# Farama-Foundation/Miniworld

Hardware: AMD Instinct MI355X
Metric: env-steps/s (batched, 80x60 RGB) (higher is better)
Workload: dtype f32

## Files before the change

include/mwengine.h:

```cpp
#ifndef MWENGINE_H
#define MWENGINE_H
#include <stdint.h>
#ifdef __cplusplus
extern "C" {
#endif

#define MW_ABI_VERSION 4

enum {
    MW_OK = 0,
    MW_E_INVALID = -1,
    MW_E_HIP = -2,
    MW_E_NOMEM = -3,
    MW_E_CAPACITY = -4,
    MW_E_DEVICE = -5,
    MW_E_OVERFLOW = -6
};

enum { MW_ENT_NONE = 0, MW_ENT_BOX = 1, MW_ENT_MESH = 2, MW_ENT_FRAME = 3 };

enum {
    MW_TASK_NONE = 0,
    MW_TASK_GOTO = 1,
    MW_TASK_PICKUP = 2,
// ... 236 lines not shown
    double cell;
    double margin;
    double reach;
    int32_t gx, gz;
    int32_t flags;
    int32_t target_slot;
} mw_nav_params;
int mw_nav_build(mw_engine *e, const mw_nav_params *params, const uint8_t *d_mask, const double *d_target, uint16_t *d_field, void *stream);
int mw_nav_query(mw_engine *e, const mw_nav_params *params, const double *d_target, const uint16_t *d_field, const double *d_pos,
                 int32_t *d_cost, int32_t *d_next, double *d_waypoint, void *stream);
int mw_debug_set_nav_passes(mw_engine *e, int32_t *d_passes);

#define MW_RAY_ENTITIES 1
#define MW_RAY_ENT 0x10000
#define MW_RAY_MAX 4096
typedef struct mw_ray_params {
    double max_t;
    double radius;
    int32_t rays;
    int32_t flags;
} mw_ray_params;
int mw_ray_cast(mw_engine *e, const mw_ray_params *params, const uint8_t *d_mask,
                const double *d_origin  ,
                const double *d_dir     ,
                const double *d_offsets ,
                double *d_t , int32_t *d_hit , double *d_dir_out ,
                void *stream);
int mw_debug_set_ray_form(mw_engine *e, int form);

#define MW_SEEN_ENTITIES 1
int mw_seen_update(mw_engine *e, const mw_nav_params *grid ,
                   const double *host_sight ,
                   int32_t flags, const uint8_t *d_mask, const uint8_t *d_clear,
                   uint8_t *d_seen, int32_t *d_count, int32_t *d_new , void *stream);

int mw_debug_set_launch_shape(mw_engine *e, int waves_per_env, int mesh_tile_waves, int ent_blocks, int slow_waves);

int mw_check(mw_engine *e, void *stream);

int mw_kernel_time_ms(mw_engine *e, int32_t reset, double *raster_ms, double *setup_ms, int64_t *launches);

int mw_get_info(mw_engine *e, int32_t *d_health, double *d_ent_pos, int32_t ent_slot, void *stream);
int mw_get_final_info(mw_engine *e, int32_t *d_health, double *d_goal_pos, void *stream);
int mw_get_reset_pending(mw_engine *e, uint8_t *d_out, void *stream);

int mw_set_frame_reuse(mw_engine *e, int32_t on);
int mw_get_frame_clean(mw_engine *e, uint8_t *d_out, void *stream);

int mw_set_frame_cache(mw_engine *e, int32_t slots);
int mw_get_frame_source(mw_engine *e, uint8_t *d_out, void *stream);
int mw_get_frame_plan(mw_engine *e, uint32_t *host_plan, int64_t words, int32_t *host_lengths, void *stream);
int mw_get_geom_built(mw_engine *e, uint8_t *host_out, void *stream);

int mw_get_list_lengths(mw_engine *e, int32_t first_env, int32_t count, int32_t *host_out, void *stream);

int mw_debug_set_mesh_frame_seq(mw_engine *e, uint32_t seq);
int mw_debug_get_slow_heads(mw_engine *e, uint32_t *host_out, void *stream);

enum { MW_PATH_TILE = 0, MW_PATH_QUAD = 1, MW_PATH_QUAD_MESH = 2, MW_PATH_GENERIC = 3 };
int mw_raster_path(const mw_engine *e);

#ifdef __cplusplus
}
#endif
#endif
```

miniworld_amd/csrc/mw_engine.h:

```cpp
#pragma once
#include <hip/hip_runtime.h>

#include <algorithm>
#include <cstdarg>
#include <cstdio>
#include <cstdlib>
#include <memory>
#include <string>
#include <utility>
#include <vector>

#include "mw_assets.h"
#include "mw_device.h"
#include "mw_kernels.h"
#include "mw_policy.h"

#define MW_TIMING_STRIDE 8

template <typename H, hipError_t (*destroy)(H)>
struct Destroy { void operator()(H h) const { (void)destroy(h); } };
template <typename T>
using DevBuf = std::unique_ptr<T, Destroy<void *, hipFree>>;
using Stream = std::unique_ptr<ihipStream_t, Destroy<hipStream_t, hipStreamDestroy>>;
using Event = std::unique_ptr<ihipEvent_t, Destroy<hipEvent_t, hipEventDestroy>>;
// ... 46 lines not shown
        uint32_t frame_seq = 1;
        DevBuf<uint32_t> slow_tris; DevBuf<float4> slow_frags; DevBuf<uint32_t> slow_head;
        DevBuf<float> plane_cache;
        int plane_cap = 0;
        int mesh_tile_waves = 16384;
        int ent_blocks = 512;
        int slow_waves = 8192;
    } mp;
    int obs_layout = MW_OBS_HWC_U8;
    float *d_reward_scratch = nullptr;
    uint8_t *d_flag_scratch = nullptr;
    uint8_t *d_mask = nullptr;
    double *d_step_override = nullptr;
    bool use_step_override = false;
    bool timing = false;
    int timing_stride = MW_TIMING_STRIDE;
    uint64_t frame_count = 0;
    struct Ev { Event a, b, c; };
    std::vector<Ev> ev_used, ev_free;
    int waves_per_env = 0;
    DevBuf<MwProgram> d_prog;
    DevBuf<mw_poly> d_prog_polys;
    DevBuf<int32_t> d_prog_room, d_prog_surf;
    DevBuf<double> d_prog_m, d_prog_segs;
    int texel_bytes = 4;
    int dbg_flags = 0;
    int last_raster_path = -1;
    bool use_k2q = true;
    bool k2q_ok = false;
    bool generic_raster = false;
    unsigned long long *d_ent_prof = nullptr;
    unsigned long long *d_k2q_prof = nullptr;
    uint8_t *final_obs = nullptr;
    float *final_depth = nullptr;
    int32_t *d_final_list = nullptr;
    const uint64_t *reset_seeds = nullptr;
    bool frame_reuse = false;
    struct { uint8_t *obs = nullptr; float *depth = nullptr; int layout = 0; bool valid = false; } held;
    struct {
        int slots = 0;
        DevBuf<uint8_t> frames;
        DevBuf<float> depth;
        DevBuf<uint64_t> meta;
        DevBuf<MwFcArgs> d_args;
        MwFcArgs args{};
        bool args_stale = true;
        bool with_depth = false;
        bool dirty = true;
    } fc;
    uint32_t *d_plan[2] = {nullptr, nullptr};
    int plan_cur = 0;
    bool geom_deal = true;
    uint8_t *d_geom_built = nullptr;
    bool plan_made = false;
    struct {
        int depth = 0, pad = 0, layout = 0, cur = 0;
        uint8_t *ring = nullptr, *final_stack = nullptr;
        size_t frame_bytes = 0;
        int64_t pushes = 0;
        uint8_t *flags = nullptr;
    } stack;
    MwSnapConfig snap_cfg{};
    MwSnapLayout snap_layout{};
    MwSnapTable *d_snap_tab = nullptr;
    int snap_chunks_per_item = 0;
    Event ev_refill_done;
};

namespace mwhost {
using namespace mwpolicy;

extern thread_local std::string g_create_error;

inline int fail(mw_engine *e, int code, const char *fmt, ...)
{
    char buf[512];
    va_list ap;
    va_start(ap, fmt);
    vsnprintf(buf, sizeof buf, fmt, ap);
    va_end(ap);
    if (e) e->err = buf; else g_create_error = buf;
    return code;
}

#define HIP_TRY(e, call)                                                                         \
    do {                                                                                         \
        hipError_t _st = (call);                                                                 \
        if (_st != hipSuccess)                                                                   \
            return fail(e, MW_E_HIP, "%s failed: %s (%s:%d)", #call, hipGetErrorString(_st), __FILE__, __LINE__); \
    } while (0)

template <typename T>
int dev_alloc(mw_engine *e, DevBuf<T> &out, size_t count, bool zero = true)
{
    void *p = nullptr;
    const size_t bytes = std::max<size_t>(count, 1) * sizeof(T);
    hipError_t st = hipMalloc(&p, bytes);
    if (st != hipSuccess) return fail(e, MW_E_NOMEM, "hipMalloc(%zu) failed: %s", bytes, hipGetErrorString(st));
    DevBuf<T> buf(static_cast<T *>(p));
    if (zero) {
        st = hipMemset(p, 0, bytes);
        if (st != hipSuccess) return fail(e, MW_E_HIP, "hipMemset failed: %s", hipGetErrorString(st));
    }
    out = std::move(buf);
    return MW_OK;
}
// ... 88 lines not shown
```

miniworld_amd/csrc/mw_engine.hip:

```cpp
#include <cmath>
#include <cstring>

#include "mw_engine.h"
#include "mw_rng.h"

namespace mwhost {
thread_local std::string g_create_error;
}
using namespace mwhost;

namespace {

void seed_env(const mw_engine *e, uint64_t *rng, int i, uint64_t seed)
{
    const size_t N = (size_t)e->cfg.num_envs;
    uint64_t w[5];
    mw::rng_seed_words(e->cfg.rng_mode == MW_RNG_PCG64, seed, w);
    for (int k = 0; k < 5; ++k) rng[(size_t)k * N + i] = w[k];
}

int upload_textures(mw_engine *e)
{
    const size_t table = (size_t)MW_MAX_TEX * sizeof(MwTexDesc) / 4;
    size_t total = table;
// ... 124 lines not shown
    a.polys = polys; a.npolys = npolys; a.segs = segs; a.nsegs = nsegs;
    MwSpare sp{};
    {
        bool want = k1_dense_lanes(cfg->max_polys, E, cfg->max_visible, cfg->task) > 0 || cfg->generator == MW_GEN_MAZE;
        if (const char *s = getenv("MW_SPARE")) want = atoi(s) != 0;
        e->spare_mode = cfg->generator != MW_GEN_NONE && !cfg->domain_rand && want && cfg->task != MW_TASK_COLLECT;
    }
    if (e->spare_mode) {
#define X(m, T, inner, slot, when, spare, view, vf) MW_WF_SPARE_##spare(MW_WF_OWNED_##when(if (rows(inner, slot, MW_WF_##when)) ALLOC(sp.m, rows(inner, slot, MW_WF_##when) * N);))
        MW_WORLD_FIELDS(X)
#undef X
        if (!cfg->shared_geometry) {
            ALLOC(sp.polys, (size_t)e->n_sets * cfg->max_polys); ALLOC(sp.npolys, e->n_sets);
            ALLOC(sp.segs, (size_t)e->n_sets * cfg->max_segs * 4); ALLOC(sp.nsegs, e->n_sets);
        }
        MwSpare *d_sp = nullptr;
        ALLOC(d_sp, 1);
        ALLOC(a.refill_mask, N);
        ALLOC(e->d_spare_dummy, 3 * (size_t)N);
        e->spare_host = sp;
        {
            std::vector<uint32_t> ones((size_t)N, 1u);
            HIP_TRY(e, hipMemcpy(a.refill_mask, ones.data(), 4 * (size_t)N, hipMemcpyHostToDevice));
        }
        HIP_TRY(e, hipMemcpy(d_sp, &sp, sizeof sp, hipMemcpyHostToDevice));
        a.spare = d_sp;
    }
    if (cfg->generator != MW_GEN_NONE) {
        ALLOC(e->d_gen_live, 1); a.gen_live = e->d_gen_live;
        if (e->spare_mode) { ALLOC(e->d_gen_spare, 1); a.gen_spare = e->d_gen_spare; }
    }
    ALLOC(e->d_meshdesc, MW_MAX_MESH);
    a.mesh = e->d_meshdesc;
    ALLOC(a.rec_raster, (size_t)N * a.max_vis * MW_RASTER_REC);
    ALLOC(a.rec_shade, (size_t)N * a.max_vis * MW_SHADE_REC);
    ALLOC(a.rec_cull, (size_t)N * a.max_vis * MW_CULL_REC);
    if (has_visiting_order(cfg->max_visible)) {
        ALLOC(a.rec_order, (size_t)N * (a.max_vis + 1));
    }
    if (cfg->max_polys > 64 && !(getenv("MW_OCC_CACHE") && atoi(getenv("MW_OCC_CACHE")) == 0)) {
        ALLOC(a.occ_valid, e->n_sets);
        ALLOC(a.occ_cache, (size_t)e->n_sets * MW_OCC_CACHE_STRIDE(cfg->max_polys));
    }
    { const auto pick = [](int id) { return id >= MW_SC_pending_remove; }; MW_WORLD_FIELDS(LIVE_ALLOC) }
    ALLOC(a.frame_clean, (size_t)N);
    ALLOC(a.fc_key, (size_t)MW_FC_KEY_WORDS * N); ALLOC(a.fc_epoch, (size_t)N); ALLOC(a.fc_source, (size_t)N);
    HIP_TRY(e, hipMemset(a.pending_remove, 0xFF, 4 * (size_t)N));
    ALLOC(a.nvis, N); ALLOC(a.envhdr, (size_t)MW_ENVHDR * N); ALLOC(a.status, 1);
    ALLOC(e->d_reward_scratch, N); ALLOC(e->d_flag_scratch, 2 * (size_t)N);
    ALLOC(e->d_final_list, 1 + (size_t)N);
    ALLOC(e->d_plan[0], MW_PLAN_WORDS(N, frame_plan_ordered(N))); ALLOC(e->d_plan[1], MW_PLAN_WORDS(N, frame_plan_ordered(N)));
    ALLOC(e->stack.flags, 2 * (size_t)N);
    ALLOC(e->d_geom_built, (size_t)N);
    ALLOC(e->d_mask, N); ALLOC(e->d_step_override, 3 * (size_t)N);
#ifdef MW_PERF_HOOKS
    if (getenv("MW_K1_PROF")) ALLOC(a.k1_prof, MW_K1_PROF_SLOTS * (size_t)N);
    if (getenv("MW_ENT_PROF")) ALLOC(e->d_ent_prof, (size_t)16 * 2 * N * MW_MAX_MESH_ENTS * 8);
    if (getenv("MW_K2Q_PROF")) ALLOC(e->d_k2q_prof, (size_t)N * 96);
#endif
#undef LIVE_ALLOC
#undef ALLOC
    {
        std::vector<int32_t> m1((size_t)N, -1);
        HIP_TRY(e, hipMemcpy(a.carry, m1.data(), 4 * (size_t)N, hipMemcpyHostToDevice));
        std::vector<uint64_t> seeds(5 * (size_t)N, 0);
        for (int i = 0; i < N; ++i) seed_env(e, seeds.data(), i, (uint64_t)i);
        HIP_TRY(e, hipMemcpy(a.rng, seeds.data(), 40 * (size_t)N, hipMemcpyHostToDevice));
    }
    e->meshes.assign(MW_MAX_MESH, {}); e->tex_desc.assign(MW_MAX_TEX, MwTexDesc{}); e->tex_data.assign(MW_MAX_TEX, {});
    if (const int rc = upload_textures(e)) return rc;
    e->waves_per_env = pick_waves_per_env(a.n_tiles, N);
#if defined(MW_PERF_HOOKS) || defined(MW_TUNE_HOOKS)
    if (const char *s = getenv("MW_WAVES_PER_ENV")) { const int v = atoi(s); if (v > 0 && a.n_tiles % v == 0) e->waves_per_env = v; }
#endif
    {
        uint32_t *p = nullptr, ids[256];
        a.n_xcc = 0;
        if (hipMalloc((void **)&p, sizeof ids) == hipSuccess) {
            const DevBuf<uint32_t> d_ids(p);
            hipLaunchKernelGGL(mw_xcc_probe_kernel, dim3(256), dim3(64), 0, 0, d_ids.get());
            if (hipMemcpy(ids, d_ids.get(), sizeof ids, hipMemcpyDeviceToHost) == hipSuccess) {
                uint32_t seen = 0u;
                for (uint32_t v : ids) seen |= 1u << (v & 15u);
                for (int n : {8, 4, 2}) if (seen == (1u << n) - 1u) a.n_xcc = n;
            }
        }
        if (a.n_xcc == 0) a.n_xcc = 1;
    }
    if (const char *s = getenv("MW_DEBUG_FLAGS")) e->dbg_flags = atoi(s) & MW_DEBUG_BITS;
    if (const char *s = getenv("MW_K2Q")) e->use_k2q = atoi(s) != 0;
    if (const char *s = getenv("MW_GENERIC_RASTER")) e->generic_raster = atoi(s) != 0;
    if (const char *s = getenv("MW_GEOM_DEAL")) e->geom_deal = atoi(s) != 0;
    e->k2q_ok = k2q_ok(cfg->msaa, a.W, a.H, mw_rasterq_lds_bytes(cfg->msaa == 4 ? 4 : 8, a.W, a.H, a.n_tiles, 1));
    {
        e->snap_cfg = {E, cfg->max_polys, cfg->max_segs, cfg->shared_geometry ? 1 : 0, cfg->task, cfg->generator, cfg->rng_mode, e->spare_mode ? 1 : 0,
                       cfg->task == MW_TASK_COLLECT ? 1 : 0};
        const MwSnapLayout &L = e->snap_layout = mw_snap_layout(e->snap_cfg);
        void *arr[MW_SC_COUNT] = {};
#define X(m, T, inner, slot, when, spare, view, vf) arr[MW_SC_##m] = (void *)a.m; MW_WF_SPARE_##spare(arr[MW_SC_SP_##m] = sp.m;)
        MW_WORLD_FIELDS(X)
#undef X
        arr[MW_SC_REFILL_MASK] = a.refill_mask;
        MwSnapTable t{};
        for (int id = 0; id < MW_SC_COUNT; ++id) {
            if (!L.comp_rows[id]) continue;
            if (!arr[id]) return fail(e, MW_E_INVALID, "snapshot layout: component %d has rows but no array", id);
            t.comp[t.n_comps++] = {arr[id], L.comp_unit[id], L.comp_row0[id], L.comp_rows[id], L.comp_elem[id], 0};
        }
        t.total_rows = L.total_rows; t.n_geo = L.n_geo; t.max_polys = cfg->max_polys; t.max_segs = cfg->max_segs;
        const int chunk = MW_SNAP_THREADS * MW_SNAP_UNROLL;
        t.poly_chunks = (cfg->max_polys * (MW_SNAP_POLY_BYTES / 16) + chunk - 1) / chunk;
        t.seg_chunks = (cfg->max_segs * (MW_SNAP_SEG_BYTES / 16) + chunk - 1) / chunk;
        t.eng_polys[0] = const_cast<mw_poly *>(a.polys); t.eng_segs[0] = const_cast<double *>(a.segs);
        t.eng_npolys[0] = const_cast<int32_t *>(a.npolys); t.eng_nsegs[0] = const_cast<int32_t *>(a.nsegs);
        t.eng_polys[1] = sp.polys; t.eng_segs[1] = sp.segs; t.eng_npolys[1] = sp.npolys; t.eng_nsegs[1] = sp.nsegs;
        t.polys_unit[0] = L.blob_unit[MW_SB_POLYS]; t.segs_unit[0] = L.blob_unit[MW_SB_SEGS];
        t.polys_unit[1] = L.blob_unit[MW_SB_SP_POLYS]; t.segs_unit[1] = L.blob_unit[MW_SB_SP_SEGS];
        t.npolys_unit[0] = L.comp_unit[MW_SC_npolys]; t.nsegs_unit[0] = L.comp_unit[MW_SC_nsegs];
        t.npolys_unit[1] = L.comp_unit[MW_SC_SP_npolys]; t.nsegs_unit[1] = L.comp_unit[MW_SC_SP_nsegs];
        t.reset_pending_unit = L.comp_unit[MW_SC_reset_pending];
        e->snap_chunks_per_item = t.n_geo * (t.poly_chunks + t.seg_chunks);
        {
            std::vector<uint16_t> row_comp((size_t)t.total_rows);
            for (int c = 0; c < t.n_comps; ++c)
                for (int r = 0; r < t.comp[c].rows; ++r) row_comp[(size_t)t.comp[c].row0 + r] = (uint16_t)c;
            uint16_t *d_row_comp = nullptr;
            if (const int rc = fixed_alloc(e, &d_row_comp, row_comp.size())) return rc;
            HIP_TRY(e, hipMemcpy(d_row_comp, row_comp.data(), row_comp.size() * sizeof(uint16_t), hipMemcpyHostToDevice));
            t.row_comp = d_row_comp;
        }
        if (const int rc = fixed_alloc(e, &e->d_snap_tab, 1)) return rc;
        HIP_TRY(e, hipMemcpy(e->d_snap_tab, &t, sizeof t, hipMemcpyHostToDevice));
    }
    return sync_gen_args(e);
}

int launch_info(mw_engine *e, int E, const int32_t *health, const double *pos, int slot, int32_t *d_health, double *d_pos, void *stream)
{
    ON_DEVICE(e);
    const int N = e->cfg.num_envs;
    hipLaunchKernelGGL(mw_info_kernel, dim3((N + 255) / 256), dim3(256), 0, (hipStream_t)stream, N, E, health, pos, slot, d_health, d_pos);
    HIP_TRY(e, hipGetLastError());
    return MW_OK;
}

// ... 418 lines not shown
}

int mw_get_list_lengths(mw_engine *e, int32_t first_env, int32_t count, int32_t *host_out, void *stream)
{
    if (!e || !host_out) return fail(e, MW_E_INVALID, "null argument");
    if (first_env < 0 || count <= 0 || first_env + count > e->cfg.num_envs) return fail(e, MW_E_INVALID, "env range out of bounds");
    ON_DEVICE(e);
    HIP_TRY(e, hipStreamSynchronize((hipStream_t)stream));
    HIP_TRY(e, hipMemcpy(host_out, e->args.nvis + first_env, sizeof(int32_t) * (size_t)count, hipMemcpyDeviceToHost));
    return MW_OK;
}

int mw_get_info(mw_engine *e, int32_t *d_health, double *d_ent_pos, int32_t ent_slot, void *stream)
{
    if (!e) return MW_E_INVALID;
    if (!d_health && !d_ent_pos) return fail(e, MW_E_INVALID, "mw_get_info: nothing asked for");
    if (d_ent_pos && (ent_slot < 0 || ent_slot >= e->args.E)) return fail(e, MW_E_INVALID, "mw_get_info: entity slot %d out of range", ent_slot);
    if (d_health && !e->args.health) return fail(e, MW_E_INVALID, "mw_get_info: this engine's task keeps no health (MW_TASK_COLLECT only)");
    return launch_info(e, e->args.E, e->args.health, e->args.epos, d_ent_pos ? ent_slot : 0, d_health, d_ent_pos, stream);
}

int mw_get_final_info(mw_engine *e, int32_t *d_health, double *d_goal_pos, void *stream)
{
    if (!e) return MW_E_INVALID;
    if (!d_health && !d_goal_pos) return fail(e, MW_E_INVALID, "mw_get_final_info: nothing asked for");
    if (d_health && !e->args.final_health) return fail(e, MW_E_INVALID, "mw_get_final_info: this engine's task keeps no health (MW_TASK_COLLECT only)");
    return launch_info(e, 1, e->args.final_health, e->args.final_goal, 0, d_health, d_goal_pos, stream);
}

int mw_get_reset_pending(mw_engine *e, uint8_t *d_out, void *stream)
{
    return e ? get_env_bytes(e, "mw_get_reset_pending", e->args.reset_pending, d_out, stream) : MW_E_INVALID;
}

int mw_get_frame_source(mw_engine *e, uint8_t *d_out, void *stream)
{
    return e ? get_env_bytes(e, "mw_get_frame_source", e->args.fc_source, d_out, stream) : MW_E_INVALID;
}

int mw_get_frame_plan(mw_engine *e, uint32_t *host_plan, int64_t words, int32_t *host_lengths, void *stream)
{
    if (!e || !host_plan || !host_lengths) return fail(e, MW_E_INVALID, "mw_get_frame_plan: null argument");
    const int N = e->cfg.num_envs;
    const size_t want = MW_PLAN_WORDS(N, frame_plan_ordered(N));
    if (words != (int64_t)want) return fail(e, MW_E_INVALID, "mw_get_frame_plan: %lld words given, the block has %zu", (long long)words, want);
    if (!e->plan_made) return fail(e, MW_E_INVALID, "mw_get_frame_plan: no frame of this engine has been planned yet");
    ON_DEVICE(e);
    HIP_TRY(e, hipStreamSynchronize((hipStream_t)stream));
    HIP_TRY(e, hipMemcpy(host_plan, e->d_plan[e->plan_cur ^ 1], want * sizeof(uint32_t), hipMemcpyDeviceToHost));
    HIP_TRY(e, hipMemcpy(host_lengths, e->args.nvis, sizeof(int32_t) * (size_t)N, hipMemcpyDeviceToHost));
    return MW_OK;
}

int mw_get_geom_built(mw_engine *e, uint8_t *host_out, void *stream)
{
    if (!e || !host_out) return fail(e, MW_E_INVALID, "mw_get_geom_built: null argument");
    ON_DEVICE(e);
    HIP_TRY(e, hipStreamSynchronize((hipStream_t)stream));
    HIP_TRY(e, hipMemcpy(host_out, e->d_geom_built, (size_t)e->cfg.num_envs, hipMemcpyDeviceToHost));
    return MW_OK;
}

int mw_get_frame_clean(mw_engine *e, uint8_t *d_out, void *stream)
{
    return e ? get_env_bytes(e, "mw_get_frame_clean", e->args.frame_clean, d_out, stream) : MW_E_INVALID;
}

int mw_kernel_time_ms(mw_engine *e, int32_t reset, double *raster_ms, double *setup_ms, int64_t *launches)
{
    if (!e) return MW_E_INVALID;
    ON_DEVICE(e);
    double r = 0, s = 0;
    int64_t n = 0;
    for (auto &ev : e->ev_used) {
        (void)hipEventSynchronize(ev.c.get());
        float t1 = 0, t2 = 0;
        (void)hipEventElapsedTime(&t1, ev.a.get(), ev.b.get());
        (void)hipEventElapsedTime(&t2, ev.b.get(), ev.c.get());
        s += t1; r += t2; ++n;
        e->ev_free.push_back(std::move(ev));
    }
    e->ev_used.clear();
    if (raster_ms) *raster_ms = n ? r / n : 0.0;
    if (setup_ms) *setup_ms = n ? s / n : 0.0;
    if (launches) *launches = n;
    e->timing = true;
    e->frame_count = 0;
    e->timing_stride = reset > 0 ? reset : MW_TIMING_STRIDE;
    if (reset < 0) e->timing = false;
    return MW_OK;
}

int mw_abi_version(void) { return MW_ABI_VERSION; }

}
```

miniworld_amd/csrc/mw_engine_frame.hip:

```cpp
#include "mw_engine.h"

using namespace mwhost;

namespace {

#define MW_K1(e, lanes, stem) ((lanes) ? MW_BY_STREAM(e, stem##_dense) : MW_BY_STREAM(e, stem))

template <typename... A>
struct KernelPair {
    void (*plain)(A...);
    void (*sub)(A..., const int32_t *);
};
template <typename... A>
KernelPair<A...> kernel_pair(void (*plain)(A...), void (*sub)(A..., const int32_t *)) { return {plain, sub}; }
#define MW_PAIR(stem) kernel_pair(stem##_kernel, stem##_sub_kernel)

template <typename... A, typename... P>
void launch(const KernelPair<A...> &k, const int32_t *list, dim3 grid, dim3 block, size_t lds, hipStream_t st, P &&...args)
{
    if (list) hipLaunchKernelGGL(k.sub, grid, block, lds, st, std::forward<P>(args)..., list);
    else hipLaunchKernelGGL(k.plain, grid, block, lds, st, std::forward<P>(args)...);
}

auto geom_kernel_of(int L, int msaa)
// ... 81 lines not shown
    int rc;
    if ((rc = grow(e, m.plane_cache, m.plane_cap, (int)want, N * (MW_PLANE_REC + MW_PLANE_XTRA) * 4))) return rc;
    if (!m.ent_list) {
        const int cap = (int)N * std::min(MW_MAX_MESH_ENTS, std::max(e->cfg.max_ents, 1));
        DevBuf<uint32_t> ents, slow, tiles;
        if ((rc = dev_alloc(e, ents, (size_t)cap * 16, false)) || (rc = dev_alloc(e, slow, N * 2, false)) ||
            (rc = dev_alloc(e, tiles, N * (size_t)a.n_tiles * 8, false)))
            return rc;
        m.ent_list_cap = cap;
        m.ent_list = std::move(ents); m.slow_envs = std::move(slow); m.tile_list = std::move(tiles);
    }
    if (!m.keys) {
        const size_t px = N * a.W * a.H;
        DevBuf<uint32_t> keys, tris, head; DevBuf<int32_t> cnt; DevBuf<float4> frags;
        if ((rc = dev_alloc(e, keys, px * 8, false)) || (rc = dev_alloc(e, cnt, N * 4 + 2 * MW_CNT_WORDS)) ||
            (rc = dev_alloc(e, tris, N * MW_SLOW_TRIS, false)) || (rc = dev_alloc(e, frags, N * MW_SLOW_STRIDE, false)) ||
            (rc = dev_alloc(e, head, px)))
            return rc;
        HIP_TRY(e, hipMemset(keys.get(), 0xFF, px * 8 * 4));
        m.ent_counter = cnt.get() + N * 4;
        m.keys = std::move(keys); m.slow_count = std::move(cnt); m.slow_tris = std::move(tris);
        m.slow_frags = std::move(frags); m.slow_head = std::move(head);
        (void)hipDeviceSynchronize();
        m.keys_dirty = false;
    }
    return MW_OK;
}

namespace {

struct MeshFrame {
    uint32_t stamp;
    int parity;
    int32_t *cnt, *cnt_next, *slow_count;
    uint32_t *slow_envs;
};
MeshFrame mesh_frame(mw_engine::MeshPath &m, size_t N)
{
    const uint32_t seq = m.frame_seq++;
    const int parity = (int)(seq & 1u);
    return {seq & 0xFFFFu, parity, m.ent_counter + parity * MW_CNT_WORDS, m.ent_counter + (parity ^ 1) * MW_CNT_WORDS,
            m.slow_count.get() + (size_t)parity * 2 * N, m.slow_envs.get() + (size_t)parity * N};
}

struct Frame {
    MwArgs a;
    int view_flags;
    const int32_t *list;
    uint8_t *obs; float *depth; hipStream_t st;
    FramePolicy pol;
    bool plans;
    RasterPath p;
    MeshFrame mf;
};

bool side_refills(const mw_engine *e) { return e->spare_mode && e->cfg.generator == MW_GEN_MAZE; }

void launch_k1(mw_engine *e, const MwArgs &ak, const Call &c, bool frameless)
{
    const int N = e->cfg.num_envs;
    const int refill_blocks = (e->spare_mode && !side_refills(e)) ? (N + 63) / 64 : 0;
    const int lanes = dense_lanes_of(e);
    const dim3 grid(env_blocks(N, lanes) + refill_blocks);
    if (c.horizon > 0 && c.trace)
        hipLaunchKernelGGL(MW_K1(e, lanes, mw_step_trace), grid, dim3(64), 0, c.st, ak, lanes, c.actions, c.reward, c.term, c.trunc, c.horizon, c.nsteps, c.step_reward,
                           frameless ? 1 : 0, *c.trace);
    else if (c.horizon > 0)
        hipLaunchKernelGGL(MW_K1(e, lanes, mw_step_plan), grid, dim3(64), 0, c.st, ak, lanes, c.actions, c.reward, c.term, c.trunc, c.horizon, c.nsteps, c.step_reward,
                           frameless ? 1 : 0);
    else if (c.repeat > 0) hipLaunchKernelGGL(MW_K1(e, lanes, mw_step_repeat), grid, dim3(64), 0, c.st, ak, lanes, c.actions, c.reward, c.term, c.trunc, c.repeat, c.nsteps);
    else hipLaunchKernelGGL(MW_K1(e, lanes, mw_step_setup), grid, dim3(64), 0, c.st, ak, lanes, c.actions, c.reward, c.term, c.trunc);
}

void launch_step_and_geometry(mw_engine *e, const Frame &f, const Call &c, CallKind kind)
{
    const MwArgs &a = f.a; const int N = e->cfg.num_envs;
    if (call_steps(kind)) {
        MwArgs ak = a;
        if (kind == CALL_TERMINAL_STEP) ak.autoreset = MW_AUTORESET_NEXT_STEP;
        launch_k1(e, ak, c, false);
    }
    if (kind == CALL_TERMINAL_STEP)
        hipLaunchKernelGGL(mw_final_list_kernel, dim3(1), dim3(1024), 0, f.st, N, (const uint8_t *)a.reset_pending, a.pending_remove, e->d_final_list);
    const int L = geom_lanes_of(e);
    const bool deals = geom_deals(f.plans, e->geom_deal, L);
    const int flags = f.view_flags | (deals ? MW_GEOM_DEAL | (f.pol.reuse ? MW_GEOM_REUSE : 0) : 0);
    launch(geom_kernel_of(L, e->cfg.msaa), f.list, dim3(env_blocks(N, L)), dim3(64), 0, f.st, a, flags, e->cfg.msaa, L, N,
           deals && f.pol.cache ? (const uint64_t *)e->fc.meta.get() : nullptr, deals && f.pol.cache ? e->fc.slots : 0, e->d_geom_built);
    if (call_steps(kind) && e->cfg.task == MW_TASK_COLLECT)
        hipLaunchKernelGGL(MW_BY_STREAM(e, mw_collect_respawn), dim3((N + 63) / 64), dim3(64), 0, f.st, a);
}

int launch_side_refill(mw_engine *e, hipStream_t st)
{
    if (!e->side_stream) HIP_TRY(e, make_stream(e->side_stream));
    if (!e->ev_fork) HIP_TRY(e, make_event(e->ev_fork));
    HIP_TRY(e, hipEventRecord(e->ev_fork.get(), st));
    HIP_TRY(e, hipStreamWaitEvent(e->side_stream.get(), e->ev_fork.get(), 0));
    hipLaunchKernelGGL(MW_BY_STREAM(e, mw_refill), dim3(e->cfg.num_envs), dim3(64), 0, e->side_stream.get(), e->args);
    e->side_refill_pending = true;
    return MW_OK;
}

int launch_generic(mw_engine *e, const MwArgs &a, int first_env, int count, int S, dim3 mesh_grid, uint8_t *out, float *depth,
                   int layout, const int32_t *list, hipStream_t st)
{
    uint32_t *keys = nullptr;
    if (e->have_meshes) {
        const size_t need = (size_t)count * a.W * a.H * S * 4;
        if (need > e->mp.view_keys_bytes) return fail(e, MW_E_INVALID, "view keys missing (mw_upload_mesh allocates them)");
        keys = e->mp.view_keys.get();
        HIP_TRY(e, hipMemsetAsync(keys, 0xFF, need, st));
        launch(MW_PAIR(mw_view_mesh), list, mesh_grid, dim3(256), 0, st, a.W, a.H, S, first_env, (const float *)a.envhdr, a.mesh_pos, keys);
    }
    const bool any = !frame_on_grid(a.W, a.H) || layout != MW_OBS_HWC_U8;
    launch(any ? MW_PAIR(mw_view_raster_any) : MW_PAIR(mw_view_raster), list, dim3(a.n_tiles, count), dim3(64), 0, st, first_env, a.W, a.H, S,
           a.max_vis, a.tiles_x, (const float *)a.rec_raster, (const float *)a.rec_shade, (const float *)a.rec_cull, (const int32_t *)a.nvis,
           (const float *)a.envhdr, a.tex, a.texels, a.mesh_pos, a.mesh_nrm, a.mesh_rgb, a.mesh_uv, keys, out, depth, e->texel_bytes, layout);
    return MW_OK;
}

void launch_quad(const mw_engine *e, const Frame &f, int part, hipStream_t st, const uint32_t *plan = nullptr)
{
    const MwArgs &a = f.a;
    const int lds = mw_rasterq_lds_bytes(e->cfg.msaa, a.W, a.H, a.n_tiles, f.depth ? 1 : 0);
    launch(f.p.quad4 ? MW_PAIR(mw_rasterq4) : MW_PAIR(mw_rasterq), f.list, dim3(e->cfg.num_envs), dim3(MWQ_THREADS), (size_t)lds, st, a.N, a.W, a.H, a.max_vis,
           a.tiles_x, a.n_tiles, (const float *)a.rec_raster, (const float *)a.rec_shade, (const float *)a.rec_cull,
           (const int32_t *)a.nvis, (const float *)a.envhdr, a.texels, f.obs, f.depth, raster_flags(e->dbg_flags, e->obs_layout, part, 0u, false), e->texel_bytes, e->d_k2q_prof,
           plan && f.pol.cache ? (const MwFcArgs *)e->fc.d_args.get() : nullptr, plan);
}

const uint32_t *launch_plan(mw_engine *e, const Frame &f, hipStream_t st)
{
    const MwArgs &a = f.a; const int N = e->cfg.num_envs;
    uint32_t *plan = e->d_plan[e->plan_cur], *next = e->d_plan[e->plan_cur ^ 1];
    e->plan_cur ^= 1;
    e->plan_made = true;
    hipLaunchKernelGGL(mw_frame_plan_kernel, dim3((N + MW_PLAN_ENVS - 1) / MW_PLAN_ENVS), dim3(64), 0, st, N, f.pol.reuse ? 1 : 0, (const uint8_t *)a.frame_clean,
                       (const uint64_t *)a.fc_key, f.pol.cache ? (const uint64_t *)e->fc.meta.get() : nullptr, f.pol.cache ? e->fc.slots : 0,
                       frame_plan_ordered(N) ? (const int32_t *)a.nvis : nullptr, a.fc_source, plan, next);
    return plan;
}

void launch_tiles(const mw_engine *e, const Frame &f, int part, hipStream_t st)
{
    const MwArgs &a = f.a; const mw_engine::MeshPath &m = e->mp;
    const TileLaunch t = tile_launch(part, a.tile_list != nullptr, f.p.big, a.max_vis, a.n_tiles, e->waves_per_env, e->cfg.num_envs, m.mesh_tile_waves);
    launch(tile_kernel_of(f.p.big, f.p.depth, f.p.general, f.p.ragged, f.p.mesh, t.part == 1), f.list, dim3(t.grid), dim3(64), t.lds, st,
           a.N, a.W, a.H, a.max_vis, a.tiles_x, a.n_tiles, t.waves_per_env, t.tiles_per_wave, (const float *)a.rec_raster, (const float *)a.rec_shade,
           (const float *)a.rec_cull, (const int32_t *)a.nvis, (const float *)a.envhdr, a.tex, a.texels, f.obs, f.depth, raster_flags(e->dbg_flags, e->obs_layout, t.part, f.mf.stamp, f.pol.reuse),
           e->texel_bytes, (const uint16_t *)a.rec_order, a.mesh_pos, a.mesh_nrm, a.mesh_rgb, a.mesh_uv, m.keys.get(),
           (const float *)m.plane_cache.get(), m.plane_cap, (const float4 *)m.slow_frags.get(), (const uint32_t *)m.slow_head.get(),
           (const uint32_t *)a.tile_list, a.ent_list_n, a.tile_list_cap, std::max(a.n_xcc, 1), (const uint8_t *)a.frame_clean);
}

int launch_mesh_chain(mw_engine *e, const Frame &f, hipStream_t st)
{
    const MwArgs &a = f.a; const MeshFrame &mf = f.mf;
    mw_engine::MeshPath &m = e->mp; const int N = e->cfg.num_envs;
    if (!m.keys || !m.plane_cache || !m.quad_stream) return fail(e, MW_E_INVALID, "mesh buffers missing (mw_upload_mesh allocates them)");
    if (m.keys_dirty) HIP_TRY(e, hipMemsetAsync(m.keys.get(), 0xFF, (size_t)N * a.W * a.H * 8 * 4, st));
    m.keys_dirty = true;
    if (mf.stamp == 0u) HIP_TRY(e, hipMemsetAsync(m.slow_head.get(), 0, (size_t)N * a.W * a.H * 4, st));
    HIP_TRY(e, hipEventRecord(m.ev_fork.get(), st));
    HIP_TRY(e, hipStreamWaitEvent(m.quad_stream.get(), m.ev_fork.get(), 0));
    hipLaunchKernelGGL(mw_mesh_entity_kernel, dim3(std::max(a.n_xcc, std::min(m.ent_list_cap, m.ent_blocks))), dim3(MW_ENT_THREADS), (size_t)e->max_mesh_verts * 16, st, N, a.W, a.H,
                       (const float *)a.envhdr, a.mesh, (const float4 *)e->pools.vpos.get(), (const uint2 *)e->pools.idx.get(), (const float *)e->pools.stream.get(),
                       (const float *)e->pools.attr.get(), m.keys.get(), m.plane_cache.get(), m.plane_cap, mf.slow_count, m.slow_tris.get(),
                       (const uint32_t *)m.ent_list.get(), m.ent_list_cap, mf.cnt, mf.cnt_next, mf.slow_envs, e->args.n_xcc, e->d_ent_prof);
    hipLaunchKernelGGL(mw_mesh_slow_kernel, dim3(std::min(N * 16, m.slow_waves)), dim3(64), 0, st, a.W, a.H, (const float *)a.envhdr, a.mesh_pos, a.mesh_nrm, a.mesh_rgb,
                       a.mesh_uv, a.texels, e->texel_bytes, m.keys.get(), m.slow_count.get(), N, mf.parity, (const uint32_t *)m.slow_tris.get(),
                       m.slow_frags.get(), m.slow_head.get(), mf.stamp, a.status,
                       (const uint32_t *)mf.slow_envs, (const int32_t *)(mf.cnt + MW_CNT_SLOW_ENVS));
    if (f.p.path == MW_PATH_QUAD_MESH) launch_quad(e, f, 1, m.quad_stream.get()); else launch_tiles(e, f, 1, m.quad_stream.get());
    launch_tiles(e, f, 2, st);
    HIP_TRY(e, hipEventRecord(m.ev_join.get(), m.quad_stream.get()));
    HIP_TRY(e, hipStreamWaitEvent(st, m.ev_join.get(), 0));
    m.keys_dirty = false;
    return MW_OK;
}

mw_engine::Ev get_events(mw_engine *e)
{
    if (!e->ev_free.empty()) {
        mw_engine::Ev ev = std::move(e->ev_free.back());
        e->ev_free.pop_back();
        return ev;
    }
    mw_engine::Ev ev;
    for (Event *x : {&ev.a, &ev.b, &ev.c}) (void)make_event(*x, hipEventDefault);
    return ev;
}

int launch_frame(mw_engine *e, const Call &c, CallKind kind, int view_flags = 0)
{
    if (!c.obs) return fail(e, MW_E_INVALID, "d_obs is null");
    uint8_t *const d_obs = c.obs; float *const d_depth = c.depth; const hipStream_t st = c.st;
    const RasterPath path = raster_path_of(e, d_depth != nullptr);
    const bool held_match = e->held.valid && e->held.obs == d_obs && e->held.depth == d_depth && e->held.layout == e->obs_layout;
    const FramePolicy pol = frame_policy({kind, view_flags, e->frame_reuse, held_match, e->have_meshes, e->dbg_flags, e->obs_layout, e->cfg.task,
                                          e->fc.slots > 0 && e->fc.frames, path.path, e->reset_seeds != nullptr});
    frames_stale(e);
    const int N = e->cfg.num_envs;
    Frame f{e->args, view_flags, kind == CALL_LIST_PASS ? e->d_final_list : nullptr, d_obs, d_depth, st, pol, false, path, {}};
    f.plans = frame_plans(pol, path.path, f.list != nullptr, N);
    if (pol.cache) {
        if (d_depth && !e->fc.depth) {
            if (const int rc = dev_alloc(e, e->fc.depth, (size_t)N * e->fc.slots * f.a.W * f.a.H, false)) return rc;
            e->fc.args_stale = true;
        }
        if ((d_depth != nullptr) != e->fc.with_depth) { e->fc.with_depth = d_depth != nullptr; e->fc.dirty = true; }
        if (e->fc.args_stale) {
            e->fc.args = MwFcArgs{f.a.fc_key, e->fc.meta.get(), e->fc.frames.get(), e->fc.depth.get(), e->fc.slots, 0};
            HIP_TRY(e, hipMemcpyAsync(e->fc.d_args.get(), &e->fc.args, sizeof(MwFcArgs), hipMemcpyHostToDevice, st));
            e->fc.args_stale = false;
            e->fc.dirty = true;
        }
        if (e->fc.dirty) {
            HIP_TRY(e, hipMemsetAsync(e->fc.meta.get(), 0, (size_t)N * MW_FC_META_WORDS(e->fc.slots) * 8, st));
            e->fc.dirty = false;
        }
    }
    f.a.step_override = e->use_step_override ? e->d_step_override : nullptr;
    if (f.p.mesh && e->mp.ent_list && e->mp.keys) {
        f.mf = mesh_frame(e->mp, (size_t)N);
        f.a.ent_list = e->mp.ent_list.get(); f.a.ent_list_n = f.mf.cnt; f.a.ent_list_cap = e->mp.ent_list_cap;
        f.a.tile_list = e->mp.tile_list.get(); f.a.tile_list_cap = N * f.a.n_tiles;
    }
    mw_engine::Ev ev{};
    const bool timed = kind != CALL_LIST_PASS && e->timing && (e->frame_count++ % (uint64_t)e->timing_stride) == 0;
    if (timed) {
        ev = get_events(e);
        (void)hipEventRecord(ev.a.get(), st);
    }
    launch_step_and_geometry(e, f, c, kind);
    if (timed) (void)hipEventRecord(ev.b.get(), st);
    int rc = MW_OK;
    if (call_steps(kind) && side_refills(e) && (rc = launch_side_refill(e, st))) return rc;
    if (f.p.path == MW_PATH_GENERIC) rc = launch_generic(e, f.a, 0, N, e->cfg.msaa, dim3(32, N), d_obs, d_depth, e->obs_layout, f.list, st);
    else if (f.p.mesh) rc = launch_mesh_chain(e, f, st);
    else if (f.p.path == MW_PATH_QUAD) launch_quad(e, f, 0, st, f.plans ? launch_plan(e, f, st) : nullptr);
    else launch_tiles(e, f, 0, st);
    if (rc) return rc;
    e->last_raster_path = f.p.path;
    if (timed) {
        (void)hipEventRecord(ev.c.get(), st);
        e->ev_used.push_back(std::move(ev));
    }
    HIP_TRY(e, hipGetLastError());
    if (pol.hold) e->held = {d_obs, d_depth, e->obs_layout, true};
    return MW_OK;
}

}

extern "C" {

static int step_passes(mw_engine *e, const Call &c, const StepPasses &p)
{
    if (p.shape == STEP_ONE_PASS) return launch_frame(e, c, CALL_STEP);
    const int N = e->cfg.num_envs;
    if (const int rc = launch_frame(e, c, CALL_TERMINAL_STEP)) return rc;
    if (p.final_copy)
        hipLaunchKernelGGL(mw_final_copy_kernel, dim3(N), dim3(256), 0, c.st, (const int32_t *)e->d_final_list, (const uint8_t *)c.obs, e->final_obs,
                           (unsigned long long)frame_bytes_of(e), (const float *)c.depth, e->final_depth, e->cfg.obs_width * e->cfg.obs_height);
    if (p.seeded_install)
        hipLaunchKernelGGL(MW_BY_STREAM(e, mw_seed_install), dim3(N), dim3(64), 0, c.st, e->args, (const int32_t *)e->d_final_list,
                           e->reset_seeds);
    else
        hipLaunchKernelGGL(MW_BY_STREAM(e, mw_final_install), dim3(N), dim3(64), 0, c.st, e->args, (const int32_t *)e->d_final_list);
    return launch_frame(e, c, CALL_LIST_PASS);
}

static int step_frameless(mw_engine *e, const Call &c)
{
    frames_stale(e);
    const int N = e->cfg.num_envs;
    MwArgs a = e->args;
    a.step_override = e->use_step_override ? e->d_step_override : nullptr;
    launch_k1(e, a, c, true);
    if (side_refills(e))
        if (const int rc = launch_side_refill(e, c.st)) return rc;
    if (e->stack.depth) {
        const ResetMode r = reset_mode(e->cfg.generator, e->cfg.autoreset);
        hipLaunchKernelGGL(mw_stack_plan_kernel, dim3((N + 255) / 256), dim3(256), 0, c.st, N, r.same ? (const uint8_t *)c.term : nullptr,
                           r.same ? (const uint8_t *)c.trunc : nullptr, r.next ? (const uint8_t *)e->args.reset_pending : nullptr, stack_flags(e, e->stack.cur));
    }
    HIP_TRY(e, hipGetLastError());
    return MW_OK;
}

static int step_frames(mw_engine *e, const char *what, Call c)
{
    ON_DEVICE(e);
    if (!c.actions) return fail(e, MW_E_INVALID, "%s: %s is null", what, c.horizon ? "d_plans" : "d_actions");
    if ((e->cfg.generator == MW_GEN_PROGRAM || e->cfg.task >= MW_TASK_SIDEWALK) && !e->args.prog)
        return fail(e, MW_E_INVALID, "no placement program installed (mw_set_gen_program)");
    const StepPasses p = step_passes_of(e->reset_seeds != nullptr, e->final_obs != nullptr, c.horizon && !c.obs);
    if (p.shape == STEP_REFUSED)
        return fail(e, MW_E_INVALID, "%s: a frameless call while reset seeds are set (mw_set_reset_seeds): the step kernel cannot seed the finished envs", what);
    resolve_outputs(e, c);
    if (p.shape == STEP_FRAMELESS) return step_frameless(e, c);
    if (const int rc = stack_check(e, what)) return rc;
    const int rc = step_passes(e, c, p);
    if (rc != MW_OK || !e->stack.depth) return rc;
    return launch_stack(e, c.obs, c.st, &c);
}

int mw_step(mw_engine *e, const int32_t *d_actions, uint8_t *d_obs, float *d_depth, float *d_reward,
            uint8_t *d_term, uint8_t *d_trunc, void *stream)
{
    if (!e) return MW_E_INVALID;
    return step_frames(e, "mw_step", Call{d_actions, d_obs, d_depth, d_reward, d_term, d_trunc, (hipStream_t)stream});
}

int mw_step_repeat(mw_engine *e, const int32_t *d_actions, int32_t repeat, uint8_t *d_obs, float *d_depth, float *d_reward,
                   uint8_t *d_term, uint8_t *d_trunc, int32_t *d_nsteps, void *stream)
{
    if (!e) return MW_E_INVALID;
    if (repeat < 1 || repeat > MW_MAX_REPEAT) return fail(e, MW_E_INVALID, "mw_step_repeat: repeat %d outside 1 .. %d", (int)repeat, MW_MAX_REPEAT);
    return step_frames(e, "mw_step_repeat", Call{d_actions, d_obs, d_depth, d_reward, d_term, d_trunc, (hipStream_t)stream, repeat, d_nsteps});
}

int mw_step_plan(mw_engine *e, const int32_t *d_plans, int32_t horizon, uint8_t *d_obs, float *d_depth, float *d_reward,
                 float *d_step_reward, uint8_t *d_term, uint8_t *d_trunc, int32_t *d_nsteps, void *stream)
{
    if (!e) return MW_E_INVALID;
    if (horizon < 1 || horizon > MW_MAX_PLAN) return fail(e, MW_E_INVALID, "mw_step_plan: horizon %d outside 1 .. %d", (int)horizon, MW_MAX_PLAN);
    if (d_depth && !d_obs) return fail(e, MW_E_INVALID, "mw_step_plan: d_depth without d_obs (a frameless call draws nothing)");
    return step_frames(e, "mw_step_plan", Call{d_plans, d_obs, d_depth, d_reward, d_term, d_trunc, (hipStream_t)stream, 0, d_nsteps, horizon, d_step_reward});
}

int mw_step_plan_trace(mw_engine *e, const int32_t *d_plans, int32_t horizon, uint8_t *d_obs, float *d_depth, float *d_reward,
// ... 60 lines not shown
    e->stack.frame_bytes = frame_bytes_of(e);
    e->stack.pushes = 0;
    return MW_OK;
}

int mw_stack_refresh(mw_engine *e, const uint8_t *d_obs, void *stream)
{
    if (!e) return MW_E_INVALID;
    if (!e->stack.depth) return fail(e, MW_E_INVALID, "mw_stack_refresh: no frame stack set (mw_set_frame_stack)");
    if (!d_obs) return fail(e, MW_E_INVALID, "mw_stack_refresh: d_obs is null");
    if (const int rc = stack_check(e, "mw_stack_refresh")) return rc;
    ON_DEVICE(e);
    return launch_stack(e, d_obs, (hipStream_t)stream, nullptr);
}

int mw_stack_window(const mw_engine *e, int32_t *first_slot, int64_t *pushes)
{
    if (!e || !e->stack.depth) return MW_E_INVALID;
    if (first_slot) *first_slot = stack_phase_of(e);
    if (pushes) *pushes = e->stack.pushes;
    return MW_OK;
}

int mw_render(mw_engine *e, uint8_t *d_obs, float *d_depth, void *stream)
{
    if (!e) return MW_E_INVALID;
    ON_DEVICE(e);
    return launch_frame(e, Call{nullptr, d_obs, d_depth, nullptr, nullptr, nullptr, (hipStream_t)stream}, CALL_RENDER);
}

int mw_render_top(mw_engine *e, uint8_t *d_obs, float *d_depth, int32_t render_agent, void *stream)
{
    if (!e) return MW_E_INVALID;
    ON_DEVICE(e);
    return launch_frame(e, Call{nullptr, d_obs, d_depth, nullptr, nullptr, nullptr, (hipStream_t)stream}, CALL_RENDER, 1 | (render_agent ? 2 : 0));
}

int mw_render_view(mw_engine *e, int32_t env, int32_t view_flags, int32_t width, int32_t height, int32_t msaa,
                   uint8_t *d_out, float *d_depth, void *stream)
{
    if (!e || !d_out) return fail(e, MW_E_INVALID, "null argument");
    ON_DEVICE(e);
    if (env < 0 || env >= e->cfg.num_envs) return fail(e, MW_E_INVALID, "env %d out of range", env);
    if (msaa != 1 && msaa != 4 && msaa != 8 && msaa != 16) return fail(e, MW_E_INVALID, "msaa must be 1, 4, 8 or 16");
    if (!frame_size_ok(width, height))
        return fail(e, MW_E_INVALID, "frame buffer size %dx%d: 1 to %d x 1 to %d pixels", width, height, 255 * MW_TILE_W, 255 * MW_TILE_H);
    frames_stale(e);
    hipStream_t st = (hipStream_t)stream;
    MwArgs b = e->args;
    b.step_override = nullptr;
    b.W = width; b.H = height;
    b.tiles_x = tiles_across(width); b.tiles_y = tiles_down(height); b.n_tiles = b.tiles_x * b.tiles_y;
    b.env_base = env;
    hipLaunchKernelGGL(geom_kernel_of(64, msaa).plain, dim3(1), dim3(64), 0, st, b, view_flags, msaa, 64, 1, (const uint64_t *)nullptr, 0, (uint8_t *)nullptr);
    if (const int rc = e->have_meshes ? grow(e, e->mp.view_keys, e->mp.view_keys_bytes, (size_t)width * height * msaa * 4, 1) : MW_OK) return rc;
    if (const int rc = launch_generic(e, b, env, 1, msaa, dim3(128), d_out, d_depth, MW_OBS_HWC_U8, nullptr, st)) return rc;
    HIP_TRY(e, hipGetLastError());
    return MW_OK;
}

int mw_set_obs_layout(mw_engine *e, int32_t layout)
{
    if (!e) return MW_E_INVALID;
    if (layout != MW_OBS_HWC_U8 && layout != MW_OBS_CWH_U8 && layout != MW_OBS_GREY_F64) return fail(e, MW_E_INVALID, "unknown obs layout %d", layout);
    world_changed(e);
    e->obs_layout = layout;
    return MW_OK;
}

int mw_visible_ents(mw_engine *e, int32_t first_env, int32_t count, uint8_t *d_vis, void *stream)
{
    if (!e || !d_vis) return fail(e, MW_E_INVALID, "null argument");
    ON_DEVICE(e);
    if (first_env < 0 || count <= 0 || first_env + count > e->cfg.num_envs) return fail(e, MW_E_INVALID, "env range out of bounds");
    const size_t lds = (size_t)e->cfg.obs_width * e->cfg.obs_height * e->cfg.msaa * 4;
    if (lds + 1024 > 160 * 1024) return fail(e, MW_E_CAPACITY, "obs frame too large for the in-LDS depth buffer of mw_visible_ents");
    hipStream_t st = (hipStream_t)stream;
    MwArgs b = e->args;
    b.step_override = nullptr;
    b.env_base = first_env;
    {
        const int L = geom_lanes_of(e);
        hipLaunchKernelGGL(geom_kernel_of(L, e->cfg.msaa).plain, dim3(env_blocks(count, L)), dim3(64), 0, st, b, 4, e->cfg.msaa, L, count, (const uint64_t *)nullptr, 0, (uint8_t *)nullptr);
    }
    if (!e->visible_attr_set) {
        HIP_TRY(e, hipFuncSetAttribute((const void *)mw_visible_kernel, hipFuncAttributeMaxDynamicSharedMemorySize, (int)lds));
        e->visible_attr_set = true;
    }
    hipLaunchKernelGGL(mw_visible_kernel, dim3(count), dim3(256), lds, st, first_env, e->cfg.obs_width, e->cfg.obs_height,
                       e->cfg.msaa, b.max_vis, e->cfg.max_ents, (const float *)b.rec_raster, (const float *)b.rec_cull, (const int32_t *)b.nvis, d_vis);
    HIP_TRY(e, hipGetLastError());
    return MW_OK;
}

int mw_set_frame_reuse(mw_engine *e, int32_t on)
{
    if (!e) return MW_E_INVALID;
    frames_stale(e);
    e->frame_reuse = on != 0;
    return MW_OK;
}

int mw_set_frame_cache(mw_engine *e, int32_t slots)
{
    if (!e) return MW_E_INVALID;
    if (slots < 0 || slots > MW_FC_MAX_SLOTS) return fail(e, MW_E_INVALID, "mw_set_frame_cache: %d slots outside 0 .. %d", (int)slots, MW_FC_MAX_SLOTS);
    ON_DEVICE(e);
    e->fc.dirty = true;
    if (slots == e->fc.slots) return MW_OK;
    HIP_TRY(e, hipDeviceSynchronize());
    e->fc.slots = 0;
    e->fc.frames.reset(); e->fc.depth.reset(); e->fc.meta.reset();
    if (slots > 0 && e->use_k2q && e->k2q_ok) {
        const size_t N = (size_t)e->cfg.num_envs;
        DevBuf<uint8_t> frames; DevBuf<uint64_t> meta;
        int rc;
        if ((rc = dev_alloc(e, frames, N * slots * e->cfg.obs_width * e->cfg.obs_height * 3, false)) || (rc = dev_alloc(e, meta, N * MW_FC_META_WORDS(slots))) ||
            (!e->fc.d_args && (rc = dev_alloc(e, e->fc.d_args, 1))))
            return rc;
        e->fc.frames = std::move(frames); e->fc.meta = std::move(meta);
        e->fc.args_stale = true;
    }
    e->fc.slots = slots;
    return MW_OK;
}

int mw_debug_set_launch_shape(mw_engine *e, int waves_per_env, int mesh_tile_waves, int ent_blocks, int slow_waves)
{
    if (!e) return MW_E_INVALID;
    if (waves_per_env < 0 || mesh_tile_waves < 0 || ent_blocks < 0 || slow_waves < 0)
        return fail(e, MW_E_INVALID, "mw_debug_set_launch_shape: negative value (%d, %d, %d, %d)", waves_per_env, mesh_tile_waves, ent_blocks, slow_waves);
    if (waves_per_env && e->args.n_tiles % waves_per_env != 0)
        return fail(e, MW_E_INVALID, "mw_debug_set_launch_shape: waves_per_env %d does not divide the %d tiles of the frame", waves_per_env, e->args.n_tiles);
    if ((mesh_tile_waves && mesh_tile_waves < 8) || (ent_blocks && ent_blocks < 8))
        return fail(e, MW_E_INVALID, "mw_debug_set_launch_shape: mesh_tile_waves %d, ent_blocks %d: fewer than 8 leave whole lists undrawn", mesh_tile_waves, ent_blocks);
    frames_stale(e);
// ... 9 lines not shown
```

miniworld_amd/csrc/mw_engine_kernels.hip:

```cpp
#include "mw_kernels.h"

extern "C" __global__ void mw_info_kernel(int N, int E, const int32_t *health, const double *epos, int slot, int32_t *out_health, double *out_pos)
{
    const int i = blockIdx.x * blockDim.x + threadIdx.x;
    if (i >= N) return;
    if (out_health) out_health[i] = health[i];
    if (out_pos)
        for (int c = 0; c < 3; ++c) out_pos[(size_t)i * 3 + c] = epos[((size_t)c * E + slot) * N + i];
}

extern "C" __global__ __launch_bounds__(1024) void mw_final_list_kernel(int N, const uint8_t *__restrict__ pending, int32_t *__restrict__ pending_remove,
                                                                       int32_t *__restrict__ list)
{
    __shared__ int s_wave[16];
    const int tid = (int)threadIdx.x, lane = tid & 63, wave = tid >> 6;
    int base = 0;
    for (int i0 = 0; i0 < N; i0 += 1024) {
        const int i = i0 + tid;
        const bool p = i < N && pending[i] != 0;
        const unsigned long long m = __ballot(p);
        if (lane == 0) s_wave[wave] = __popcll(m);
        __syncthreads();
        int before = base, total = 0;
        for (int w = 0; w < 16; ++w) {
            const int c = s_wave[w];
            before += w < wave ? c : 0;
            total += c;
        }
        if (p) {
            list[1 + before + __popcll(m & ((1ull << lane) - 1ull))] = i;
            pending_remove[i] = -1;
        }
        base += total;
        __syncthreads();
    }
    if (tid == 0) list[0] = base;
}

extern "C" __global__ __launch_bounds__(256) void mw_final_copy_kernel(const int32_t *__restrict__ list, const uint8_t *__restrict__ obs,
                                                                      uint8_t *__restrict__ final_obs, unsigned long long row_bytes,
                                                                      const float *__restrict__ depth, float *__restrict__ final_depth, int depth_row)
{
    if ((int)blockIdx.x >= list[0]) return;
    const size_t env = (size_t)list[1 + blockIdx.x];
    const uint8_t *src = obs + env * row_bytes;
    uint8_t *dst = final_obs + env * row_bytes;
    if ((((uintptr_t)obs | (uintptr_t)final_obs | (uintptr_t)row_bytes) & 15u) == 0) {
        for (size_t k = threadIdx.x; k < row_bytes / 16; k += blockDim.x)
            reinterpret_cast<uint4 *>(dst)[k] = reinterpret_cast<const uint4 *>(src)[k];
    } else {
        for (size_t k = threadIdx.x; k < row_bytes; k += blockDim.x) dst[k] = src[k];
    }
    if (depth && final_depth)
        for (int k = threadIdx.x; k < depth_row; k += blockDim.x) final_depth[env * depth_row + k] = depth[env * depth_row + k];
}

extern "C" __global__ __launch_bounds__(64) void mw_frame_plan_kernel(int N, int reuse, const uint8_t *__restrict__ frame_clean, const uint64_t *__restrict__ key,
                                                                     const uint64_t *__restrict__ meta, int slots, const int32_t *__restrict__ nvis,
                                                                     uint8_t *__restrict__ frame_source, uint32_t *__restrict__ plan, uint32_t *__restrict__ next)
{
    const int lane = (int)threadIdx.x, env = (int)blockIdx.x * MW_PLAN_ENVS + lane;
    const bool ordered = nvis != nullptr;
    if (blockIdx.x == 0) {
        if (lane < 2) next[lane] = 0u;
        else if (lane < 4) next[MW_PLAN_CLS_LO + lane - 2] = 0u;
        else if (lane < 6) next[MW_PLAN_CLS_HI + lane - 4] = 0u;
        else if (lane == 6) plan[2] = ordered ? (uint32_t)MW_PLAN_CLASSES : 0u;
    }
    const bool on = env < N;
    uint32_t v = MW_SRC_CLEAN;
    uint32_t cls = 0u;
    if (on) {
        const bool clean = frame_clean[env] != 0;
        const int32_t len = ordered ? nvis[env] : 0;
        uint32_t match = 0u, header = 0u;
        if (meta) {
            const uint64_t *row = static_cast<const uint64_t *>(__builtin_assume_aligned(meta + (size_t)env * MW_FC_META_WORDS(slots), 16));
            const uint64_t *cur = static_cast<const uint64_t *>(__builtin_assume_aligned(key + (size_t)env * MW_FC_KEY_WORDS, 16));
            header = (uint32_t)row[0];
#pragma unroll
            for (int j = 0; j < MW_FC_MAX_SLOTS; ++j) {
                const int jj = j < slots ? j : slots - 1;
                match |= mw_fc_key_equal(static_cast<const uint64_t *>(__builtin_assume_aligned(row + 2 + MW_FC_KEY_WORDS * jj, 16)), cur) && j < slots ? 1u << j : 0u;
            }
        }
        v = mw_frame_verdict(clean, reuse != 0, match, header, meta ? slots : 0);
        frame_source[env] = (uint8_t)v;
        cls = mw_plan_cost_class(len);
    }
    const uint32_t src = v & 0xFFu;
    const bool draw = on && src == MW_SRC_DRAWN, copy = on && src >= (uint32_t)MW_SRC_SLOT(0);
    const uint64_t md = __builtin_amdgcn_ballot_w64(draw), mc = __builtin_amdgcn_ballot_w64(copy), below = (1ull << lane) - 1ull;
    unsigned long long add = (unsigned long long)__popcll(md) | (unsigned long long)__popcll(mc) << 32, add_lo = 0ull, add_hi = 0ull;
    uint64_t mine = md;
    if (ordered) {
#pragma unroll
        for (uint32_t c = 0; c < MW_PLAN_CLASSES; ++c) {
            const uint64_t m = __builtin_amdgcn_ballot_w64(draw && cls == c);
            (c < 4u ? add_lo : add_hi) |= (unsigned long long)__popcll(m) << (16u * (c & 3u));
            mine = cls == c ? m : mine;
        }
    }
    unsigned long long old = 0ull;
    if (lane < 3) {
        const unsigned long long a = lane == 0 ? add : lane == 1 ? add_lo : add_hi;
        uint32_t *at = plan + (lane == 0 ? 0 : lane == 1 ? MW_PLAN_CLS_LO : MW_PLAN_CLS_HI);
        if (a) old = atomicAdd(reinterpret_cast<unsigned long long *>(at), a);
    }
    const uint32_t old_lo = (uint32_t)old, old_hi = (uint32_t)(old >> 32);
    const uint32_t bd = (uint32_t)__builtin_amdgcn_readlane((int)old_lo, 0), bc = (uint32_t)__builtin_amdgcn_readlane((int)old_hi, 0);
    const uint64_t base_lo = (uint64_t)(uint32_t)__builtin_amdgcn_readlane((int)old_lo, 1) | (uint64_t)(uint32_t)__builtin_amdgcn_readlane((int)old_hi, 1) << 32;
    const uint64_t base_hi = (uint64_t)(uint32_t)__builtin_amdgcn_readlane((int)old_lo, 2) | (uint64_t)(uint32_t)__builtin_amdgcn_readlane((int)old_hi, 2) << 32;
    const uint32_t entry = (uint32_t)env | (v >> 8) << MW_PLAN_ENV_BITS;
    const uint32_t id = (ordered ? mw_plan_class_count(base_lo, base_hi, cls) : bd) + (uint32_t)__popcll(mine & below), ic = bc + (uint32_t)__popcll(mc & below);
    if (draw && id < (uint32_t)N) plan[MW_PLAN_DRAW(N, ordered ? cls : 0u) + id] = entry;
    if (copy && ic < (uint32_t)N) plan[MW_PLAN_COPY(N) + ic] = entry;
}
```

miniworld_amd/csrc/mw_geom.hip:

```cpp
#include <cstddef>
#include "mw_setup_common.h"
#include "mw_records.h"
#include "mw_kernels.h"
#include "mw_geom_deal.h"

namespace {

constexpr int kClipSlots = 24;

__device__ inline void wave_lds_sync()
{
    __builtin_amdgcn_fence(__ATOMIC_RELEASE, "workgroup", "local");
    __builtin_amdgcn_wave_barrier();
    __builtin_amdgcn_fence(__ATOMIC_ACQUIRE, "workgroup", "local");
}

constexpr int kDealStageSlots = 4;
constexpr int kDealStageQuads = 64 * (MW_FC_META_WORDS(kDealStageSlots) / 2);
__device__ inline uint64_t deal_mask(const uint8_t *__restrict__ frame_clean, const int32_t *__restrict__ pending_remove, const uint64_t *__restrict__ fc_key,
                                     const uint64_t *__restrict__ meta, int slots, bool reuse, int env0, int n, int lane, uint4 *stage)
{
    const bool on = lane < n;
    const int env = env0 + (on ? lane : 0);
    const bool clean = frame_clean[env] != 0;
// ... 122 lines not shown
    const int g0 = (b0 + 15) >> 4, g1 = (b1 + 1) >> 4;
    if (g0 >= g1) {
        for (int b = b0; b <= b1; ++b)
            if (!(occ_z[b] < thr)) return false;
        return true;
    }
    for (int b = b0; b < (g0 << 4); ++b)
        if (!(occ_z[b] < thr)) return false;
    for (int g = g0; g < g1; ++g)
        if (!(occ_z[MW_OCC_BINS + g] < thr)) return false;
    for (int b = g1 << 4; b <= b1; ++b)
        if (!(occ_z[b] < thr)) return false;
    return true;
}

__device__ inline bool occluded(const float *occ_z, const mwgl::Vert v[4], float bins_per_px)
{
    float zq = 1e30f, xmn = 1e30f, xmx = -1e30f;
    bool ok = true;
#pragma unroll
    for (int k = 0; k < 4; ++k) {
        ok &= v[k].clip[3] >= 0.1f;
        xmn = fminf(xmn, v[k].win[0]); xmx = fmaxf(xmx, v[k].win[0]); zq = fminf(zq, v[k].clip[3]);
    }
    return ok && occluded_span(occ_z, xmn - 0.1f, xmx + 0.1f, zq, bins_per_px);
}

__device__ inline bool occluded_span_rmq(const float *rmq, float xlo, float xhi, float zq, float bins_per_px)
{
    const float fb0 = floorf(fmaxf(xlo, 0.0f) * bins_per_px), fb1 = floorf(fmaxf(xhi, 0.0f) * bins_per_px);
    const int b0 = (int)fminf(fb0, (float)(MW_OCC_BINS - 1)), b1 = (int)fminf(fb1, (float)(MW_OCC_BINS - 1));
    const float thr = zq * __builtin_amdgcn_rcpf(fmaf(1.2e-3f, zq, 1.0f)) * 0.9999f;
    if (b1 < b0) return true;
    const int k = 31 - __builtin_clz((unsigned)(b1 - b0 + 1));
    const float m = fmaxf(rmq[k * MW_OCC_BINS + b0], rmq[k * MW_OCC_BINS + b1 - (1 << k) + 1]);
    return m < thr;
}

__device__ inline bool occluded_rmq(const float *rmq, const mwgl::Vert v[4], float bins_per_px)
{
    float zq = 1e30f, xmn = 1e30f, xmx = -1e30f;
    bool ok = true;
#pragma unroll
    for (int k = 0; k < 4; ++k) {
        ok &= v[k].clip[3] >= 0.1f;
        xmn = fminf(xmn, v[k].win[0]); xmx = fmaxf(xmx, v[k].win[0]); zq = fminf(zq, v[k].clip[3]);
    }
    return ok && occluded_span_rmq(rmq, xmn - 0.1f, xmx + 0.1f, zq, bins_per_px);
}

}

template <bool BIG, int SFIX, bool SUB = false>
__device__ inline void geom_body(const MwArgs &a, int view_flags, int S_, int L, int n_env, const uint64_t *fc_meta, int fc_slots, uint8_t *built, const int32_t *__restrict__ list = nullptr)
{
    const int S = SFIX ? SFIX : S_;
    struct ClipSlot { mwgl::ClipVert l[2][MWGL_MAX_CLIP_VERTS]; float pad[4]; };
    __shared__ ClipSlot s_clip[kClipSlots];
    static_assert(BIG || (alignof(ClipSlot) >= 16 && sizeof(ClipSlot) * kClipSlots >= kDealStageQuads * sizeof(uint4)), "the dealing prologue borrows the clipper's LDS");
    __shared__ int s_pos[BIG ? 1 : 8][66];
    __shared__ uint32_t s_meta[64], s_res[64];
    __shared__ float s_occ_z[BIG ? MW_OCC_BINS + MW_OCC_BINS / 16 : 1];
    __shared__ int s_occ_n;
    float *s_rmq = reinterpret_cast<float *>(&s_clip[0]);
    float4 *s_occ_wall = reinterpret_cast<float4 *>(s_rmq + 9 * MW_OCC_BINS);
    static_assert(!BIG || sizeof(ClipSlot) * kClipSlots >= (9 * MW_OCC_BINS + 8 * MW_OCC_CAP) * sizeof(float), "the sift borrows the clipper's LDS");
    __shared__ uint16_t s_list[BIG ? 4096 : 1];
    __shared__ uint32_t s_key[BIG ? MW_ORDER_CAP : 1];
#ifdef MW_PERF_HOOKS
#define KGP_ON (a.k1_prof != nullptr)
#else
#define KGP_ON false
#endif
    const unsigned long long tstart = KGP_ON ? __builtin_readcyclecounter() : 0ull;
    const unsigned long long rt_start = KGP_ON ? __builtin_amdgcn_s_memrealtime() : 0ull;
    [[maybe_unused]] unsigned long long ts[4] = {0, 0, 0, 0};
    [[maybe_unused]] int kp_nocc = 0, kp_nkept = 0, kp_nclip = 0;
    [[maybe_unused]] unsigned long long kp_clip = 0, kp_emit = 0, kp_e_shfl = 0, kp_e_setup = 0, kp_e_write = 0;
    const int lane = threadIdx.x;
    const int epw = 64 / L, sub = lane & (L - 1), grp = lane / L;
    const bool deal = !BIG && !SUB && (view_flags & MW_GEOM_DEAL) != 0;
    int rel, env;
    bool live;
    constexpr bool kPoseAhead = !BIG && !SUB;
    constexpr int kPoseWords = 17;
    [[maybe_unused]] double ahead[kPoseWords];
    [[maybe_unused]] int ahead_lane = 0;
    if constexpr (BIG) {
        if (SUB) {
            n_env = list[0];
            if ((int)blockIdx.x * epw >= n_env) return;
        }
        rel = (int)blockIdx.x * epw + grp;
        live = rel < n_env;
        env = SUB ? list[1 + (live ? rel : n_env - 1)] : a.env_base + (live ? rel : n_env - 1);
    } else {
        if (SUB) n_env = list[0];
        const int lg = __ffs(L) - 1, g = (int)blockIdx.x >> lg, i = (int)blockIdx.x & (L - 1);
        const int waves = min(L, (int)gridDim.x - (g << lg));
        const int mine = 64 * g + lane;
        if (kPoseAhead) {
            const int ge = a.env_base + min(mine, n_env - 1);
            ahead[0] = a.ax[ge]; ahead[1] = a.ay[ge]; ahead[2] = a.az[ge]; ahead[3] = a.adir[ge];
#pragma unroll
            for (int i = 0; i < 9; ++i) ahead[4 + i] = a.light[(size_t)(3 + i) * a.N + ge];
#pragma unroll
            for (int i = 0; i < 4; ++i) ahead[13 + i] = a.cam[(size_t)i * a.N + ge];
        }
        uint64_t mask;
        if (deal) mask = deal_mask(a.frame_clean, a.pending_remove, a.fc_key, fc_meta, fc_slots, (view_flags & MW_GEOM_REUSE) != 0, a.env_base + 64 * g, n_env - 64 * g, lane, reinterpret_cast<uint4 *>(&s_clip[0]));
        else mask = __ballot(mine < n_env);
        const bool want = ((mask >> lane) & 1ull) != 0ull;
        if (deal && i == 0 && mine < n_env && !want) built[a.env_base + mine] = 0;
        if ((int)__popcll((unsigned long long)mask) <= i) return;
        const int bit = mw_geom_deal(mask, waves, i, grp);
        live = bit >= 0;
        rel = 64 * g + (live ? bit : mw_geom_deal(mask, waves, i, 0));
        env = SUB ? list[1 + rel] : a.env_base + rel;
        ahead_lane = rel - 64 * g;
    }
    if (kPoseAhead) {
#pragma unroll
        for (int i = 0; i < kPoseWords; ++i) ahead[i] = __shfl(ahead[i], ahead_lane);
    }
    const int set = a.shared_geom ? 0 : env;
    const bool top = (view_flags & 1) != 0, proxy = (view_flags & 4) != 0, ms = S > 1;
    constexpr int kWallPf = BIG ? 4 : 1;
    float4 pf_wall[kWallPf], pf_box0 = make_float4(0.0f, 0.0f, 0.0f, 0.0f), pf_box1 = pf_box0;
    float pf_sgn[kWallPf], pf_hdr[3] = {0.0f, 0.0f, 0.0f};
    auto prefetch_occ = [&]() {
        if (!BIG || L != 64 || a.occ_cache == nullptr) return;
        const float *pc = a.occ_cache + (size_t)set * MW_OCC_CACHE_STRIDE(a.max_polys);
#pragma unroll
        for (int q = 0; q < kWallPf; ++q) {
            const int i = lane + 64 * q;
            if (i < a.max_polys) {
                pf_wall[q] = reinterpret_cast<const float4 *>(pc + MW_OCC_CACHE_HDR + 8 * (size_t)i)[0];
                pf_sgn[q] = pc[MW_OCC_CACHE_HDR + 8 * (size_t)i + 4];
            }
        }
        if (lane < (a.max_polys + 7) / 8) {
            const float4 *b4 = reinterpret_cast<const float4 *>(pc + MW_OCC_CACHE_HDR + 8 * (size_t)a.max_polys + 8 * (size_t)lane);
            pf_box0 = b4[0]; pf_box1 = b4[1];
        }
        pf_hdr[0] = pc[0]; pf_hdr[1] = pc[1]; pf_hdr[2] = pc[2];
    };
#pragma unroll
    for (int q = 0; q < kWallPf; ++q) { pf_wall[q] = make_float4(0.0f, 0.0f, 0.0f, 0.0f); pf_sgn[q] = 0.0f; }
    prefetch_occ();
    const bool ent_pre = a.E <= L;
    const int my_ekind = (ent_pre && sub < a.E && (BIG || live)) ? a.ekind[(size_t)sub * a.N + env] : 0;
    const int my_estatic = (ent_pre && sub < a.E) ? a.estatic[(size_t)sub * a.N + env] : 0;
    const int my_emesh = (ent_pre && sub < a.E && my_ekind == MW_ENT_MESH) ? a.emesh[(size_t)sub * a.N + env] : 0;
    const int my_mesh_ntris = (ent_pre && sub < a.E && my_ekind == MW_ENT_MESH) ? (int)a.mesh[my_emesh].ntris : 0;
    auto ent_kind = [&](int s0) { return ent_pre ? __shfl(my_ekind, s0, L) : (BIG || live) ? a.ekind[(size_t)s0 * a.N + env] : (int)MW_ENT_NONE; };
    auto ent_static = [&](int s0) { return ent_pre ? __shfl(my_estatic, s0, L) : a.estatic[(size_t)s0 * a.N + env]; };
    auto ent_mesh_ntris = [&](int s0) { return ent_pre ? __shfl(my_mesh_ntris, s0, L) : (int)a.mesh[a.emesh[(size_t)s0 * a.N + env]].ntris; };
    mwgl::Frame f;
    const double px = kPoseAhead ? ahead[0] : a.ax[env], py = kPoseAhead ? ahead[1] : a.ay[env], pz = kPoseAhead ? ahead[2] : a.az[env], dir = kPoseAhead ? ahead[3] : a.adir[env];
    float eye_x = 0.0f, eye_y = 0.0f, eye_z = 0.0f;
    {
        double lpos[3], lcol[3], lamb[3];
#pragma unroll
// ... 582 lines not shown
            bool box_clipped = clipped_l;
            if (is_box) {
                const int fc = (item - npd) % 6;
                const int first = lane - (2 * fc + tsel);
                const bool whole = sub - (2 * fc + tsel) >= 0 && sub - (2 * fc + tsel) + 11 < L;
                if (whole) {
                    box_clipped = ((cm >> first) & 0xFFFull) != 0ull;
                } else {
                    box_clipped = false;
                }
                if (!whole) {
                    const int slot = box_slot;
                    const double ex_ = a.epos[((size_t)0 * a.E + slot) * a.N + env], ey_ = a.epos[((size_t)1 * a.E + slot) * a.N + env],
                                 ez_ = a.epos[((size_t)2 * a.E + slot) * a.N + env];
                    float lo[3], hi[3];
                    mwgl::Xform ex;
                    const mwgl::Xform *x = &cam;
                    if (proxy) {
                        lo[0] = (float)(ex_ - 0.1); lo[1] = (float)ey_; lo[2] = (float)(ez_ - 0.1);
                        hi[0] = (float)(ex_ + 0.1); hi[1] = (float)(ey_ + 0.2); hi[2] = (float)(ez_ + 0.1);
                    } else {
                        const float pos[3] = {(float)ex_, (float)ey_, (float)ez_};
                        mwgl::entity_xform(f, pos, (float)(a.edir[(size_t)slot * a.N + env] * (180 / kPi)), 1.0f, false, ex);
                        x = &ex;
                        const double sx = a.egeom[((size_t)0 * a.E + slot) * a.N + env], sy = a.egeom[((size_t)1 * a.E + slot) * a.N + env],
                                     sz = a.egeom[((size_t)2 * a.E + slot) * a.N + env];
                        lo[0] = (float)(-sx / 2); lo[1] = 0.0f; lo[2] = (float)(-sz / 2);
                        hi[0] = (float)(sx / 2); hi[1] = (float)sy; hi[2] = (float)(sz / 2);
                    }
                    for (int c = 0; c < 8; ++c) {
                        const float p[3] = {(c & 1) ? hi[0] : lo[0], (c & 2) ? hi[1] : lo[1], (c & 4) ? hi[2] : lo[2]};
                        mwgl::Vert o;
                        mwgl::transform_vertex(f, *x, p, o);
                        box_clipped |= o.clipmask != 0u;
                    }
                }
                direct = !box_clipped && !in_list;
            }
        }

        KGP_R(2);
        if (KGP_ON) { if (rnd == 0) rvert[0] = tprev - rstart; rvert[1] = tprev - rstart; }
        const mwgl::Vert va = tsel ? (direct ? v[0] : v[1]) : v[0], vb = tsel ? v[2] : v[1], vc = tsel ? v[3] : (direct ? v[2] : v[3]);
        int cnt = 0;
        bool clipped = false;
        if (tsel < nt && !(va.clipmask & vb.clipmask & vc.clipmask)) {
            if ((va.clipmask | vb.clipmask | vc.clipmask) == 0u) cnt = tri_front(va.win, vb.win, vc.win, ms) ? 1 : 0;
            else clipped = true;
        }
        KGP_R(3);
        const uint64_t cmask = __ballot(clipped);
        const uint64_t below = (1ull << lane) - 1ull;
        const int n_clip = (int)__popcll((unsigned long long)cmask);
        const bool keep_lists = n_clip <= kClipSlots;
        const uint32_t cm_union = va.clipmask | vb.clipmask | vc.clipmask;
        const bool par = !__any(clipped && __popc(cm_union) == 6);
        mwgl::ClipVert *kept = nullptr;
        int kept_n = 0;
        const int cg0 = lane & ~7, ce = lane & 7;
        const int my_v = (int)__popcll((unsigned long long)(cmask & below));
        auto clip_lists = [&](int v0) {
            if (clipped && my_v >= v0 && my_v < v0 + kClipSlots) {
                ClipSlot &cs = s_clip[my_v - v0];
                mwgl::clip_copy_in(cs.l[0][0], va); mwgl::clip_copy_in(cs.l[0][1], vb); mwgl::clip_copy_in(cs.l[0][2], vc);
            }
            wave_lds_sync();
            const int nb = n_clip - v0 < kClipSlots ? n_clip - v0 : kClipSlots;
            for (int b0 = 0; b0 < nb; b0 += 8) {
                const int slot = b0 + (lane >> 3);
                const bool valid = slot < nb;
                ClipSlot &cs = s_clip[valid ? slot : 0];
                uint32_t cm = valid ? s_meta[v0 + slot] >> 8 : 0u;
                int n = valid ? 3 : 0, cur = 0;
                while (__any(cm != 0u && n >= 3)) {
                    const bool act = cm != 0u && n >= 3;
                    const int plane = act ? __ffs((int)cm) - 1 : 0;
                    if (act) cm &= cm - 1u;
                    const mwgl::ClipVert *in = cs.l[cur];
                    mwgl::ClipVert *out = cs.l[cur ^ 1];
                    const bool me = act && ce < n;
                    const int nxt = ce + 1 < n ? ce + 1 : 0;
                    mwgl::ClipVert V;
                    if (me) V = in[ce];
                    const float dp_prev = me ? mwgl::clip_dist(V, plane) : 0.0f;
                    const float dp = __shfl(dp_prev, cg0 + nxt);
                    const bool bad = me && (!(dp_prev == dp_prev) || dp_prev - dp_prev != 0.0f);
                    const bool emit = me && dp_prev >= 0.0f, cross = me && ((dp >= 0.0f) != (dp_prev >= 0.0f));
                    const uint32_t bg = (uint32_t)(__ballot(bad) >> cg0) & 0xFFu;
                    const uint32_t eg = (uint32_t)(__ballot(emit) >> cg0) & 0xFFu, xg = (uint32_t)(__ballot(cross) >> cg0) & 0xFFu;
                    const uint32_t lowm = (1u << ce) - 1u;
                    const int pos = __popc(eg & lowm) + __popc(xg & lowm);
                    if (emit) out[pos] = V;
                    if (cross) {
                        const mwgl::ClipVert Vn = in[nxt];
                        const bool from_cur = fabsf(dp) < fabsf(dp_prev);
                        const float t = (from_cur ? dp : dp_prev) / (from_cur ? dp - dp_prev : dp_prev - dp);
                        mwgl::clip_interp<false>(f, out[pos + (emit ? 1 : 0)], t, from_cur ? Vn : V, from_cur ? V : Vn);
                    }
                    if (act) { n = bg ? 0 : __popc(eg) + __popc(xg); cur ^= 1; }
                    wave_lds_sync();
                }
                if (n < 3) n = 0;
                const mwgl::ClipVert *r = cs.l[cur];
                bool front = false;
                if (ce >= 2 && ce < n) front = tri_front(r[ce - 1].win, r[ce].win, r[0].win, ms);
                const uint32_t fm = (uint32_t)(__ballot(front) >> cg0) & 0xFFu;
// ... 97 lines not shown
                    if (!keep_lists) {
                        const int slot = (int)__popcll((unsigned long long)(batch & below));
                        mwgl::ClipVert *r2;
                        n = mwgl::clip_triangle<false>(f, va, vb, vc, s_clip[slot].l[0], s_clip[slot].l[1], &r2);
                        r = r2;
                    }
                    int idx = base;
                    for (int i = 2; i < n; ++i) {
                        mwgl::TriSetup t2;
                        if (mwgl::setup_triangle(to_vert(r[i - 1], va.col), to_vert(r[i], va.col), to_vert(r[0], va.col), ms, tex >= 0, t2)) {
                            if (live && idx < a.max_vis) {
                                const uint32_t zlo = (SFIX == 8 ? mwrec::write_tri_s<8>(a, env, idx, tag ? tag : (uint32_t)idx + id_base, t2, tex) : mwrec::write_tri(a, env, idx, tag ? tag : (uint32_t)idx + id_base, t2, tex, S));
                                if (BIG && idx < MW_ORDER_CAP) s_key[idx] = (zlo << 16) | (uint32_t)idx;
                            }
                            ++idx;
                        }
                    }
                }
                pend = rest;
            }
        }
        KGP_R(6);
        if (KGP_ON && rnd < 2) rtot[rnd] = tprev - rstart;
        if (is_box && tsel == 0 && (item - npd) % 6 == 0 && (item - npd) / 6 < 64) pos[(item - npd) / 6] = base;
        if (marker && tsel == 0 && item == n_items - 1) pos[total_boxes < 64 ? total_boxes : 64] = base;
    }
    wave_lds_sync();
    if (BIG && a.rec_order && L < 64) {
        if (sub == 0 && live) a.rec_order[(size_t)env * (a.max_vis + 1)] = 0;
    } else if (BIG && a.rec_order) {
        uint16_t *order = a.rec_order + (size_t)env * (a.max_vis + 1);
        const int n = count;
        if (n > MW_ORDER_CAP || n > a.max_vis || !live) {
            if (lane == 0 && live) order[0] = 0;
        } else {
            wave_lds_sync();
            if (n <= 64) sort_store_keys<1>(s_key, n, lane, order);
            else if (n <= 128) sort_store_keys<2>(s_key, n, lane, order);
            else if (n <= 256) sort_store_keys<4>(s_key, n, lane, order);
            else sort_store_keys<8>(s_key, n, lane, order);
            if (lane == 0) order[0] = 1;
        }
    }
    if (KGP_ON && sub == 0 && live) {
        unsigned long long *pp = a.k1_prof + (size_t)env * MW_K1_PROF_SLOTS;
        pp[0] = tp[0] - tstart; pp[1] = tp[1] - tp[0]; for (int i = 2; i < 7; ++i) pp[i] = racc[i];
        pp[7] = __builtin_readcyclecounter() - tprev;
        pp[20] = rtot[0]; pp[21] = rtot[1]; pp[22] = rvert[0]; pp[23] = rvert[1];
        pp[24] = kp_clip; pp[25] = kp_emit; pp[26] = (unsigned long long)kp_nclip; pp[27] = 0; pp[28] = kp_e_shfl; pp[29] = kp_e_setup; pp[30] = kp_e_write;
        pp[8] = rt_start; pp[9] = __builtin_amdgcn_s_memrealtime();
        pp[10] = (unsigned long long)np; pp[11] = (unsigned long long)npd; pp[12] = (unsigned long long)count; pp[13] = (unsigned long long)n_rounds;
        pp[14] = (unsigned long long)kp_nocc; pp[15] = (unsigned long long)kp_nkept;
        pp[16] = ts[0] - tp[0]; pp[17] = ts[1] - ts[0]; pp[18] = ts[2] - ts[1]; pp[19] = ts[3] - ts[2];
    }
    if (ent_pre && my_mesh_j >= 0 && live) {
        const int nb = total_boxes < 64 ? total_boxes : 64;
        const int end_pos = marker ? pos[nb] : count;
        const int p0 = my_boxes_before < nb ? pos[my_boxes_before] : end_pos;
        hdr[MW_HDR_MESH + MW_HDR_MESH_STRIDE * my_mesh_j + 1] = __int_as_float(p0 + my_tris_before);
    }
    if (sub == 0 && live) {
        if (deal) built[env] = 1;
        a.nvis[env] = count < a.max_vis ? count : a.max_vis;
        hdr[0] = (float)a.light[(size_t)0 * a.N + env]; hdr[1] = (float)a.light[(size_t)1 * a.N + env]; hdr[2] = (float)a.light[(size_t)2 * a.N + env];
        hdr[3] = __int_as_float(total_meshes);
#pragma unroll
        for (int i = 0; i < 3; ++i) { hdr[4 + i] = f.l_amb[i]; hdr[8 + i] = f.l_dif[i]; }
        const int nb = total_boxes < 64 ? total_boxes : 64;
        const int end_pos = marker ? pos[nb] : count;
        if (!ent_pre) {
            for (int j = 0; j < total_meshes; ++j) {
                float *m = hdr + MW_HDR_MESH + MW_HDR_MESH_STRIDE * j;
                const int before = __float_as_int(m[1]);
                const int p0 = before < nb ? pos[before] : end_pos;
                m[1] = __int_as_float(p0 + __float_as_int(m[25]));
            }
        }
        if (count + total_mesh_tris >= 0xFFF0) atomicOr(a.status, MW_ST_VIS_OVERFLOW);
        if (a.ent_list && total_meshes > 0) {
            const int nbig = __popc(big_mask);
            const int xl = env % a.n_xcc;
            int ib = nbig ? atomicAdd(a.ent_list_n + MW_CNT_LONG + xl, nbig) : 0;
            int is = total_meshes - nbig ? atomicAdd(a.ent_list_n + MW_CNT_SHORT + xl, total_meshes - nbig) : 0;
            uint32_t *l_long = a.ent_list + (size_t)xl * a.ent_list_cap, *l_short = a.ent_list + (size_t)(8 + xl) * a.ent_list_cap;
            for (int j = 0; j < total_meshes; ++j) {
                const uint32_t item = (uint32_t)env | ((uint32_t)j << 24);
                if ((big_mask >> j) & 1u) { if (ib < a.ent_list_cap) l_long[ib] = item; ++ib; }
                else { if (is < a.ent_list_cap) l_short[is] = item; ++is; }
            }
        }
        const int rs = a.pending_remove[env];
        if (rs >= 0 && !proxy && a.task != MW_TASK_COLLECT) {
            a.ekind[(size_t)rs * a.N + env] = MW_ENT_NONE;
            a.pending_remove[env] = MW_REMOVE_APPLIED;
        }
    }
    if (a.tile_list) {
        int total;
        const int cnt = live ? __popc(tile_mask) : 0, excl = group_excl_scan(cnt, sub, L, total);
        int o = 0;
        const int xl = env % a.n_xcc;
        if (sub == 0 && total > 0) o = atomicAdd(a.ent_list_n + MW_CNT_TILES + xl, total);
        o = __shfl(o, 0, L) + excl;
        uint32_t *list = a.tile_list + (size_t)xl * a.tile_list_cap;
        for (uint32_t m = live ? tile_mask : 0u; m; m &= m - 1u, ++o)
            if (o < a.tile_list_cap) list[o] = (uint32_t)env | ((uint32_t)(sub + (__ffs((int)m) - 1) * L) << 24);
    }
}

#ifndef MW_GEOM_OCC
#define MW_GEOM_OCC
#endif
#define MW_GEOM_PAIR(stem, bounds, ...)                                                                                        \
    extern "C" __global__ bounds void stem##_kernel(MW_GEOM_ARGS) { geom_body<__VA_ARGS__, false>(a, view_flags, S, L, n_env, fc_meta, fc_slots, built); } \
    extern "C" __global__ bounds void stem##_sub_kernel(MW_GEOM_ARGS, const int32_t *list) { geom_body<__VA_ARGS__, true>(a, view_flags, S, L, n_env, fc_meta, fc_slots, built, list); }
MW_GEOM_PAIR(mw_geom, __launch_bounds__(64) MW_GEOM_OCC, false, 8)
MW_GEOM_PAIR(mw_geom_big, __launch_bounds__(64) MW_GEOM_OCC, true, 8)
MW_GEOM_PAIR(mw_geom_any, __launch_bounds__(64), false, 0)
MW_GEOM_PAIR(mw_geom_big_any, __launch_bounds__(64), true, 0)

extern "C" __global__ __launch_bounds__(64) void mw_selftest_sort_kernel(const uint32_t *keys, const int32_t *n, uint16_t *order)
{
    __shared__ uint32_t s_key[MW_ORDER_CAP];
    const int lane = threadIdx.x, cnt = n[blockIdx.x];
    for (int i = lane; i < cnt; i += 64) s_key[i] = keys[(size_t)blockIdx.x * MW_ORDER_CAP + i];
    __syncthreads();
    uint16_t *out = order + (size_t)blockIdx.x * (MW_ORDER_CAP + 1);
    if (cnt <= 64) sort_store_keys<1>(s_key, cnt, lane, out);
    else if (cnt <= 128) sort_store_keys<2>(s_key, cnt, lane, out);
    else if (cnt <= 256) sort_store_keys<4>(s_key, cnt, lane, out);
    else sort_store_keys<8>(s_key, cnt, lane, out);
}

extern "C" int mw_selftest_sort(const uint32_t *host_keys , const int32_t *host_n , int32_t blocks, uint16_t *host_order )
{
    uint32_t *d_keys = nullptr; int32_t *d_n = nullptr; uint16_t *d_order = nullptr;
    const size_t kb = (size_t)blocks * MW_ORDER_CAP * 4, ob = (size_t)blocks * (MW_ORDER_CAP + 1) * 2;
    if (blocks <= 0 || hipMalloc((void **)&d_keys, kb) != hipSuccess || hipMalloc((void **)&d_n, (size_t)blocks * 4) != hipSuccess ||
        hipMalloc((void **)&d_order, ob) != hipSuccess) return -1;
    (void)hipMemcpy(d_keys, host_keys, kb, hipMemcpyHostToDevice);
    (void)hipMemcpy(d_n, host_n, (size_t)blocks * 4, hipMemcpyHostToDevice);
    (void)hipMemset(d_order, 0, ob);
    hipLaunchKernelGGL(mw_selftest_sort_kernel, dim3(blocks), dim3(64), 0, 0, d_keys, d_n, d_order);
    const int rc = hipDeviceSynchronize() == hipSuccess ? 0 : -2;
    (void)hipMemcpy(host_order, d_order, ob, hipMemcpyDeviceToHost);
    (void)hipFree(d_keys); (void)hipFree(d_n); (void)hipFree(d_order);
    return rc;
}
```

miniworld_amd/csrc/mw_kernels.h:

```cpp
#pragma once
#include "mw_device.h"
#include "mw_frame_plan.h"
#include "mw_snapshot.h"
#include "mw_snapframes.h"
#include "mw_state_view.h"
#include "mw_nav.h"
#include "mw_ray.h"
#include "mw_seen.h"

#define MW_KERNEL_PAIR(stem, ...)                          \
    extern "C" __global__ void stem##_kernel(__VA_ARGS__); \
    extern "C" __global__ void stem##_sub_kernel(__VA_ARGS__, const int32_t *list)

#define MW_RNG_PAIR(stem, ...)                             \
    extern "C" __global__ void stem##_kernel(__VA_ARGS__); \
    extern "C" __global__ void stem##_pcg_kernel(__VA_ARGS__)
#define MW_CAT_(a, b) a##b
#define MW_CAT(a, b) MW_CAT_(a, b)
#define MW_STREAM_SUFFIX_0
#define MW_STREAM_SUFFIX_1 _pcg
#define MW_KERNEL_NAME(stem) MW_CAT(MW_CAT(stem, MW_CAT(MW_STREAM_SUFFIX_, MW_RNG_KIND)), _kernel)

#define MW_K1_DECLARE(stem, ...) MW_RNG_PAIR(stem, __VA_ARGS__); MW_RNG_PAIR(stem##_dense, __VA_ARGS__)
#define MW_K1_STEM(stem, ...) stem
#define MW_K1_PARAMS_OF(stem, ...) __VA_ARGS__
#define MW_K1_ARGS MwArgs a, int lanes_per_env, const int32_t *__restrict__ actions, float *__restrict__ reward, \
                   uint8_t *__restrict__ term, uint8_t *__restrict__ trunc
#define MW_K1_ROW_0(X) X(mw_step_setup, MW_K1_ARGS)
MW_K1_ROW_0(MW_K1_DECLARE);
#define MW_K1_REPEAT_ARGS MW_K1_ARGS, int repeat, int32_t *__restrict__ nsteps
#define MW_K1_ROW_1(X) X(mw_step_repeat, MW_K1_REPEAT_ARGS)
MW_K1_ROW_1(MW_K1_DECLARE);
#define MW_K1_PLAN_ARGS MW_K1_ARGS, int horizon, int32_t *__restrict__ nsteps, float *__restrict__ step_reward, int frameless
#define MW_K1_ROW_2(X) X(mw_step_plan, MW_K1_PLAN_ARGS)
MW_K1_ROW_2(MW_K1_DECLARE);
#define MW_K1_TRACE_ARGS MW_K1_PLAN_ARGS, mw_plan_trace trace
#define MW_K1_ROW_3(X) X(mw_step_trace, MW_K1_TRACE_ARGS)
MW_K1_ROW_3(MW_K1_DECLARE);

MW_RNG_PAIR(mw_reset, MwArgs a, const uint8_t *__restrict__ mask, int force_all, int mark_refill);
MW_RNG_PAIR(mw_refill, MwArgs a);
MW_RNG_PAIR(mw_collect_respawn, MwArgs a);
MW_RNG_PAIR(mw_final_install, MwArgs a, const int32_t *__restrict__ list);
extern "C" __global__ void mw_take_spare_kernel(MwArgs a, const uint8_t *__restrict__ mask, int force_all);
MW_RNG_PAIR(mw_reset_where, MwArgs a, const uint8_t *__restrict__ mask, const uint64_t *__restrict__ seeds);
MW_RNG_PAIR(mw_seed_install, MwArgs a, const int32_t *__restrict__ list, const uint64_t *__restrict__ next_seed);

#define MW_GEOM_DEAL 8
#define MW_GEOM_REUSE 16
#define MW_GEOM_ARGS MwArgs a, int view_flags, int S, int L, int n_env, const uint64_t *fc_meta, int fc_slots, uint8_t *built
MW_KERNEL_PAIR(mw_geom, MW_GEOM_ARGS);
MW_KERNEL_PAIR(mw_geom_big, MW_GEOM_ARGS);
MW_KERNEL_PAIR(mw_geom_any, MW_GEOM_ARGS);
MW_KERNEL_PAIR(mw_geom_big_any, MW_GEOM_ARGS);


#define MW_RASTER_ARGS \
    int N, int W, int H, int max_vis, int tiles_x, int n_tiles, int waves_per_env, int tiles_per_wave, \
    const float *__restrict__ rec_raster, const float *__restrict__ rec_shade, const float *__restrict__ rec_cull, \
    const int32_t *__restrict__ nvis_arr, const float *__restrict__ envhdr, const MwTexDesc *__restrict__ texd, \
    const uint32_t *__restrict__ texels, uint8_t *__restrict__ obs, float *__restrict__ depth, int dbg, int texel_bytes, \
    const uint16_t *__restrict__ rec_order, const float *__restrict__ mesh_pos, const float *__restrict__ mesh_nrm, \
    const float *__restrict__ mesh_rgb, const float *__restrict__ mesh_uv, uint32_t *__restrict__ mesh_keys, \
    const float *__restrict__ plane_cache, int plane_cap, const float4 *__restrict__ slow_frags, const uint32_t *__restrict__ slow_head, \
    const uint32_t *__restrict__ tile_list, int32_t *__restrict__ tile_n, int tile_list_cap, int n_xcc, \
    const uint8_t *__restrict__ frame_clean
MW_KERNEL_PAIR(mw_raster, MW_RASTER_ARGS);
MW_KERNEL_PAIR(mw_raster_depth, MW_RASTER_ARGS);
MW_KERNEL_PAIR(mw_raster_big, MW_RASTER_ARGS);
MW_KERNEL_PAIR(mw_raster_big_depth, MW_RASTER_ARGS);
MW_KERNEL_PAIR(mw_raster_wrap, MW_RASTER_ARGS);
MW_KERNEL_PAIR(mw_raster_big_wrap, MW_RASTER_ARGS);
MW_KERNEL_PAIR(mw_raster_ragged, MW_RASTER_ARGS);
MW_KERNEL_PAIR(mw_raster_big_ragged, MW_RASTER_ARGS);
MW_KERNEL_PAIR(mw_raster_nomesh, MW_RASTER_ARGS);
MW_KERNEL_PAIR(mw_raster_nomesh_depth, MW_RASTER_ARGS);
MW_KERNEL_PAIR(mw_raster_mesh, MW_RASTER_ARGS);
MW_KERNEL_PAIR(mw_raster_mesh_depth, MW_RASTER_ARGS);
MW_KERNEL_PAIR(mw_raster_mesh_wrap, MW_RASTER_ARGS);
MW_KERNEL_PAIR(mw_raster_big_mesh_wrap, MW_RASTER_ARGS);

#define MWQ_THREADS 512
#define MWQ_ARGS \
    int N, int W, int H, int max_vis, int tiles_x, int n_tiles, \
    const float *__restrict__ rec_raster, const float *__restrict__ rec_shade, const float *__restrict__ rec_cull, \
    const int32_t *__restrict__ nvis_arr, const float *__restrict__ envhdr, const uint32_t *__restrict__ texels, \
    uint8_t *__restrict__ obs, float *__restrict__ depth, int dbg, int texel_bytes, unsigned long long *__restrict__ prof, \
    const MwFcArgs *__restrict__ fc, const uint32_t *__restrict__ plan
MW_KERNEL_PAIR(mw_rasterq, MWQ_ARGS);
MW_KERNEL_PAIR(mw_rasterq4, MWQ_ARGS);
extern "C" int mw_rasterq_lds_bytes(int S, int W, int H, int n_tiles, int depth);
extern "C" int mw_rasterq_cap(int depth);

extern "C" __global__ void mw_mesh_entity_kernel(
    int N, int W, int H, const float *__restrict__ envhdr, const MwMeshDesc *__restrict__ meshes, const float4 *__restrict__ mesh_vpos,
    const uint2 *__restrict__ mesh_idx, const float *__restrict__ mesh_stream, const float *__restrict__ mesh_attr, uint32_t *__restrict__ keys_all,
    float *__restrict__ plane_cache, int plane_cap, int32_t *__restrict__ slow_count, uint32_t *__restrict__ slow_tris, const uint32_t *__restrict__ ent_list,
    int ent_list_cap, int32_t *ent_n, int32_t *ent_n_after, uint32_t *__restrict__ slow_envs, int n_xcc, unsigned long long *prof);
extern "C" __global__ void mw_mesh_slow_kernel(int W, int H, const float *envhdr, const float *mesh_pos, const float *mesh_nrm, const float *mesh_rgb,
                                               const float *mesh_uv, const uint32_t *texels, int texel_bytes, uint32_t *keys, int32_t *counts, int N,
                                               int parity, const uint32_t *slow_tris, float4 *frags, uint32_t *heads, uint32_t stamp, uint32_t *status,
                                               const uint32_t *slow_envs, const int32_t *slow_env_n);
extern "C" __global__ void mw_xcc_probe_kernel(uint32_t *out);

MW_KERNEL_PAIR(mw_view_mesh, int W, int H, int S, int first_env, const float *__restrict__ envhdr, const float *__restrict__ mesh_pos, uint32_t *keys);
#define MW_VIEW_RASTER_ARGS \
    int first_env, int W, int H, int S, int max_vis, int tiles_x, const float *__restrict__ rec_raster, \
    const float *__restrict__ rec_shade, const float *__restrict__ rec_cull, const int32_t *__restrict__ nvis_arr, const float *__restrict__ envhdr, \
    const MwTexDesc *__restrict__ texd, const uint32_t *__restrict__ texels, const float *__restrict__ mesh_pos, \
    const float *__restrict__ mesh_nrm, const float *__restrict__ mesh_rgb, const float *__restrict__ mesh_uv, const uint32_t *mesh_keys, \
    uint8_t *__restrict__ out, float *__restrict__ depth, int texel_bytes, int layout
MW_KERNEL_PAIR(mw_view_raster, MW_VIEW_RASTER_ARGS);
MW_KERNEL_PAIR(mw_view_raster_any, MW_VIEW_RASTER_ARGS);

#define MW_STACK_FRESH 1
#define MW_STACK_PENDING 2
#define MW_STACK_ARGS \
    int depth, int pad, int phase, unsigned long long frame_bytes, int wide, const uint8_t *__restrict__ obs, uint8_t *ring, \
    const uint8_t *__restrict__ flags_in, uint8_t *__restrict__ flags_out
extern "C" __global__ void mw_stack_push_kernel(MW_STACK_ARGS, const uint8_t *__restrict__ term, const uint8_t *__restrict__ trunc,
                                                const uint8_t *__restrict__ pending, const uint8_t *__restrict__ final_obs,
                                                uint8_t *__restrict__ final_stack);
extern "C" __global__ void mw_stack_refresh_kernel(MW_STACK_ARGS);
extern "C" __global__ void mw_stack_mark_kernel(int N, const uint8_t *__restrict__ mask, int force_all, uint8_t *__restrict__ flags);
extern "C" __global__ void mw_stack_plan_kernel(int N, const uint8_t *__restrict__ term, const uint8_t *__restrict__ trunc,
                                                const uint8_t *__restrict__ pending, uint8_t *__restrict__ flags);

#define MW_SNAP_ITEMS const int32_t *__restrict__ d_envs, const int32_t *__restrict__ d_recs, const uint8_t *__restrict__ mask
#define MW_SNAP_ARGS \
    const MwSnapTable *__restrict__ tab, MwSnapKey key, int N, int capacity, int count, int item_chunks, uint32_t *__restrict__ status
extern "C" __global__ void mw_snapshot_save_kernel(MW_SNAP_ARGS, uint8_t *__restrict__ snap, MW_SNAP_ITEMS);
extern "C" __global__ void mw_snapshot_load_kernel(MW_SNAP_ARGS, const uint8_t *__restrict__ snap, int n_recs, uint8_t *__restrict__ frame_clean,
                                                   int32_t *__restrict__ occ_valid, uint8_t *__restrict__ stack_flags, uint32_t *__restrict__ fc_epoch,
                                                   MW_SNAP_ITEMS);

#define MW_SNAPF_ARGS MwSnapfArgs a, uint32_t *__restrict__ status
extern "C" __global__ void mw_snapshot_save_frames_kernel(MW_SNAPF_ARGS, const uint8_t *__restrict__ obs, const uint8_t *__restrict__ depth,
                                                          const uint8_t *__restrict__ ring, const uint8_t *__restrict__ stack_flags,
                                                          uint8_t *__restrict__ frames, MW_SNAP_ITEMS);
extern "C" __global__ void mw_snapshot_load_frames_kernel(MW_SNAPF_ARGS, const uint8_t *__restrict__ frames, uint8_t *__restrict__ obs,
                                                          uint8_t *__restrict__ depth, uint8_t *__restrict__ ring, uint8_t *__restrict__ stack_flags,
                                                          MW_SNAP_ITEMS);

extern "C" __global__ void mw_info_kernel(int N, int E, const int32_t *health, const double *epos, int slot, int32_t *out_health, double *out_pos);
extern "C" __global__ void mw_final_list_kernel(int N, const uint8_t *__restrict__ pending, int32_t *__restrict__ pending_remove, int32_t *__restrict__ list);
extern "C" __global__ void mw_final_copy_kernel(const int32_t *__restrict__ list, const uint8_t *__restrict__ obs, uint8_t *__restrict__ final_obs,
                                                unsigned long long row_bytes, const float *__restrict__ depth, float *__restrict__ final_depth, int depth_row);
#define MW_PLAN_ENVS 64
extern "C" __global__ void mw_frame_plan_kernel(int N, int reuse, const uint8_t *__restrict__ frame_clean, const uint64_t *__restrict__ key,
                                                const uint64_t *__restrict__ meta, int slots, const int32_t *__restrict__ nvis,
                                                uint8_t *__restrict__ frame_source, uint32_t *__restrict__ plan, uint32_t *__restrict__ next);

#define MW_SV_THREADS 256
#define MW_SV_ENVS (MW_SV_THREADS / 64)
extern "C" __global__ void mw_state_get_kernel(MwStateArrays a, mw_state_view v, int N, int E, int first_env, int count);
extern "C" __global__ void mw_state_set_where_kernel(MwStateArrays a, mw_state_view v, const uint8_t *__restrict__ mask, int N, int E,
                                                     uint32_t *__restrict__ status, uint8_t *__restrict__ reset_pending,
                                                     uint8_t *__restrict__ frame_clean, uint32_t *__restrict__ fc_epoch,
                                                     uint8_t *__restrict__ stack_flags);

#define MW_NAV_THREADS 512
#define MW_NAV_QUERY_THREADS 256
extern "C" __global__ void mw_nav_build_kernel(MwNavArgs a, mw_nav_params p, const uint8_t *__restrict__ mask, const double *__restrict__ d_target,
                                               uint16_t *__restrict__ field, int32_t *__restrict__ passes);
extern "C" __global__ void mw_nav_query_kernel(MwNavArgs a, mw_nav_params p, const double *__restrict__ d_target, const uint16_t *__restrict__ field,
                                               const double *__restrict__ pos, int32_t *__restrict__ cost, int32_t *__restrict__ next,
                                               double *__restrict__ waypoint);

extern "C" __global__ void mw_ray_lanes_kernel(MwRayArgs a, mw_ray_params p, const uint8_t *__restrict__ mask, const double *__restrict__ origin,
                                               const double *__restrict__ dir, const double *__restrict__ offsets, double *__restrict__ t_out,
                                               int32_t *__restrict__ hit_out, double *__restrict__ dir_out);
extern "C" __global__ void mw_ray_waves_kernel(MwRayArgs a, mw_ray_params p, const uint8_t *__restrict__ mask, const double *__restrict__ origin,
                                               const double *__restrict__ dir, const double *__restrict__ offsets, double *__restrict__ t_out,
                                               int32_t *__restrict__ hit_out, double *__restrict__ dir_out);

extern "C" __global__ void mw_seen_kernel(MwRayArgs a, mw_nav_params p, mwseen::Sight s, const uint8_t *__restrict__ mask, const uint8_t *__restrict__ clear,
                                          uint8_t *seen, int32_t *__restrict__ count, int32_t *__restrict__ newly);

extern "C" __global__ void mw_visible_kernel(int env_base, int W, int H, int S, int max_vis, int E, const float *__restrict__ rec_raster,
                                             const float *__restrict__ rec_cull, const int32_t *__restrict__ nvis, uint8_t *__restrict__ vis);
```

miniworld_amd/csrc/mw_policy.h:

```cpp
#pragma once
#include <stddef.h>
#include <stdint.h>

#include "../../include/mwengine.h"
#include "mw_ray.h"
#include "mw_seen.h"
#include "mw_shape.h"
#include "mw_snapframes.h"
#include "mw_snapshot.h"

namespace mwpolicy {

inline bool tile_kernels_exact(int W, int H) { return W <= 128 && H <= 128 && W * H <= 128 * 96; }

inline int tiles_across(int W) { return (W + MW_TILE_W - 1) / MW_TILE_W; }
inline int tiles_down(int H) { return (H + MW_TILE_H - 1) / MW_TILE_H; }
inline bool frame_on_grid(int W, int H) { return W % MW_TILE_W == 0 && H % MW_TILE_H == 0; }
inline bool tile_path_ok(int W, int H) { return frame_on_grid(W, H) && tile_kernels_exact(W, H); }
inline bool frame_size_ok(int W, int H) { return W >= 1 && H >= 1 && W <= 255 * MW_TILE_W && H <= 255 * MW_TILE_H; }

inline bool has_visiting_order(int max_visible) { return max_visible > 64; }

inline int geom_lanes(int max_polys, int max_ents, bool order)
{
// ... 69 lines not shown
struct ResetMode { bool installs, same, next; };
inline ResetMode reset_mode(int generator, int autoreset)
{
    const bool installs = generator != MW_GEN_NONE;
    return {installs, installs && autoreset == MW_AUTORESET_SAME_STEP, installs && autoreset == MW_AUTORESET_NEXT_STEP};
}

enum CallKind { CALL_RENDER = 0, CALL_STEP = 1, CALL_TERMINAL_STEP = 2, CALL_LIST_PASS = 3 };
inline bool call_steps(CallKind k) { return k == CALL_STEP || k == CALL_TERMINAL_STEP; }

enum StepShape { STEP_REFUSED = -1, STEP_FRAMELESS = 0, STEP_ONE_PASS = 1, STEP_TWO_PASS = 2 };
struct StepPasses { StepShape shape; bool final_copy, seeded_install; };
inline StepPasses step_passes_of(bool seeds, bool final_bufs, bool frameless)
{
    if (frameless) return {seeds ? STEP_REFUSED : STEP_FRAMELESS, false, false};
    if (!seeds && !final_bufs) return {STEP_ONE_PASS, false, false};
    return {STEP_TWO_PASS, final_bufs, seeds};
}

struct FrameFacts {
    CallKind kind;
    int view_flags;
    bool frame_reuse, held_match;
    bool meshes;
    int dbg_flags, layout, task;
    bool cache_allocated;
    int path;
    bool seeded = false;
};
struct FramePolicy {
    bool reuse;
    bool source;
    bool cache;
    bool hold;
};
inline FramePolicy frame_policy(const FrameFacts &f)
{
    const bool plain = (f.kind == CALL_RENDER || f.kind == CALL_STEP) && f.view_flags == 0;
    const bool seeded_pass = f.seeded && (f.kind == CALL_TERMINAL_STEP || f.kind == CALL_LIST_PASS) && f.view_flags == 0;
    const bool plain_step = (plain && f.kind == CALL_STEP) || (seeded_pass && f.kind == CALL_TERMINAL_STEP), bare = !f.meshes && f.dbg_flags == 0;
    const bool source = plain_step && f.path == MW_PATH_QUAD;
    return {f.frame_reuse && plain_step && bare && f.held_match, source,
            source && f.cache_allocated && bare && f.layout == MW_OBS_HWC_U8 && f.task != MW_TASK_COLLECT, plain || seeded_pass};
}

inline bool frame_plans(const FramePolicy &pol, int path, bool listed, int N)
{
    return !listed && path == MW_PATH_QUAD && (pol.reuse || pol.cache) && N <= 0xFFFFFF;
}
inline bool geom_deals(bool plans, bool enabled, int lanes)
{
    return plans && enabled && lanes < 64;
}
inline bool frame_plan_ordered(int N)
{
    return N <= 0xFFFF;
}

struct TileLaunch { int part, waves_per_env, tiles_per_wave, grid; size_t lds; };
inline TileLaunch tile_launch(int part, bool tile_list, bool big, int max_vis, int n_tiles, int wpe, int N, int mesh_tile_waves)
{
    const int lds_recs = max_vis < MW_LDS_RECS ? max_vis : MW_LDS_RECS;
    const size_t lds = big ? 192 : (size_t)lds_recs * (MW_LDS_SHADE_Q + MW_LDS_CULL_Q) * 16 + 192;
    const bool listed = part == 2 && tile_list;
    if (listed) part = 3;
    const int wpe2 = part == 2 ? n_tiles : wpe, tpw2 = part == 2 ? 1 : (n_tiles + wpe - 1) / wpe;
    const int all = N * n_tiles;
    return {part, wpe2, tpw2, listed ? (mesh_tile_waves < all ? mesh_tile_waves : all) : (N + 7) / 8 * 8 * wpe2, lds};
}

inline bool wide_units(uintptr_t bits) { return (bits & 15u) == 0; }

struct StackLaunch { bool wide; unsigned chunks; };
inline StackLaunch stack_launch(uintptr_t address_bits, size_t frame_bytes)
{
    const bool wide = wide_units(address_bits | (uintptr_t)frame_bytes);
    const size_t units = frame_bytes / (wide ? 16 : 1), chunk = (size_t)MW_STACK_THREADS * MW_STACK_UNROLL;
    return {wide, (unsigned)((units + chunk - 1) / chunk)};
}

inline bool grid_too_large(unsigned long long blocks) { return blocks > 0x7FFFFFFFull; }

struct SnapshotGrid { int item_chunks; long long blocks; };
inline SnapshotGrid snapshot_grid(int count, int total_rows, int chunks_per_item)
{
    const int item_chunks = (count + MW_SNAP_THREADS - 1) / MW_SNAP_THREADS;
    return {item_chunks, (long long)item_chunks * total_rows + (long long)count * chunks_per_item};
}

inline SnapshotGrid snapshot_where_grid(int N, int total_rows, int chunks_per_item) { return snapshot_grid(N, total_rows, chunks_per_item); }

struct LoadInvalidation { bool held, cache; };
inline LoadInvalidation snapshot_load_invalidation(bool where) { return {true, !where}; }
inline LoadInvalidation reset_where_invalidation() { return snapshot_load_invalidation(true); }
inline LoadInvalidation set_state_where_invalidation() { return snapshot_load_invalidation(true); }
inline LoadInvalidation snapshot_load_frames_invalidation(bool ) { return {true, false}; }

struct SnapfGrid { bool wide; uint64_t frame_chunks, depth_chunks, per_item, blocks; };
inline SnapfGrid snapf_grid(uintptr_t address_bits, uint64_t frame_bytes, uint64_t depth_bytes, int stack_depth, int count)
{
    const bool wide = wide_units(address_bits | (uintptr_t)frame_bytes | (uintptr_t)depth_bytes);
    const uint64_t chunk = (uint64_t)MW_SNAPF_THREADS * MW_SNAPF_UNROLL * (wide ? 16 : 1);
    const uint64_t frame_chunks = (frame_bytes + chunk - 1) / chunk, depth_chunks = (depth_bytes + chunk - 1) / chunk;
    const uint64_t per_item = frame_chunks * (1 + (uint64_t)stack_depth) + depth_chunks;
    return {wide, frame_chunks, depth_chunks, per_item, per_item * (uint64_t)count};
}
// ... 26 lines not shown
```

miniworld_amd/csrc/mw_setup.hip:

```cpp
#include "mw_setup_common.h"
#include "mw_kernels.h"

#ifndef MW_K1_OCC
#define MW_K1_OCC 3
#endif

extern "C" __global__ __launch_bounds__(64) __attribute__((amdgpu_waves_per_eu(MW_K1_OCC, 4))) void MW_K1_NAME()(
    MW_K1_PARAMS)
{
    __shared__ int s_claim;
    __shared__ unsigned char gen_ws[MW_GEN_WS_BYTES];
    if ((int)blockIdx.x >= a.N) {
        mw::refill_spares(a, (int)blockIdx.x - a.N, (int)threadIdx.x, gen_ws);
        return;
    }
    const int lane = threadIdx.x & 63;
    MW_K1_STEP(false, a.env_base + (int)blockIdx.x, lane, lane == 0, gen_ws, &s_claim);
}
```

miniworld_amd/csrc/mw_setup_common.h:

```cpp
#pragma once
#include "mw_device.h"
#include "mw_math.h"
#include "mw_rng.h"
#include "mw_gen.h"

namespace {

constexpr double kPi = 3.14159265358979323846;

__device__ inline uint64_t ballot(bool p) { return __ballot(p); }

__device__ inline float uni(float v) { return __int_as_float(__builtin_amdgcn_readfirstlane(__float_as_int(v))); }
__device__ inline int uni(int v) { return __builtin_amdgcn_readfirstlane(v); }
__device__ inline double uni(double v)
{
    const unsigned long long b = (unsigned long long)__double_as_longlong(v);
    const unsigned lo = (unsigned)__builtin_amdgcn_readfirstlane((int)(unsigned)b);
    const unsigned hi = (unsigned)__builtin_amdgcn_readfirstlane((int)(unsigned)(b >> 32));
    return __longlong_as_double((long long)(((unsigned long long)hi << 32) | lo));
}

__device__ inline bool same_bits(double x, double y) { return __double_as_longlong(x) == __double_as_longlong(y); }

__device__ inline void store_frame_key(const MwArgs &a, int env, double px, double py, double pz, double dir, int carry, uint32_t epoch,
                                       double cx, double cy, double cz, double cdir)
{
    ulonglong2 *k = reinterpret_cast<ulonglong2 *>(a.fc_key + (size_t)env * MW_FC_KEY_WORDS);
    auto bits = [](double v) { return (unsigned long long)__double_as_longlong(v); };
    const bool c = carry >= 0;
    k[0] = make_ulonglong2(bits(px), bits(py));
    k[1] = make_ulonglong2(bits(pz), bits(dir));
    k[2] = make_ulonglong2((unsigned long long)(uint32_t)carry | ((unsigned long long)epoch << 32), c ? bits(cx) : 0ull);
    k[3] = make_ulonglong2(c ? bits(cy) : 0ull, c ? bits(cz) : 0ull);
    k[4] = make_ulonglong2(c ? bits(cdir) : 0ull, 1ull);
}


struct StepCtx {
    const MwArgs &a;
    int env, lane, set;
    double px, py, pz, dir;
    double cam_height;
    int carry;
    int live;
    double cpos[3], cdir;
};

__device__ inline double ent_pos(const StepCtx &c, int slot, int comp)
{
    if (slot == c.live) return c.cpos[comp];
    return c.a.epos[((size_t)comp * c.a.E + slot) * c.a.N + c.env];
}

__device__ inline double ent_geom(const MwArgs &a, int env, int slot, int k)
{
    return a.egeom[((size_t)k * a.E + slot) * a.N + env];
}

using mw::radii_sum;
__device__ inline bool is_mesh(const MwArgs &a, int env, int slot) { return a.ekind[(size_t)slot * a.N + env] == MW_ENT_MESH; }

__device__ int intersect_wave(const StepCtx &c, int self_slot, double x, double z, double radius)
{
    const MwArgs &a = c.a;
    const double *segs = a.segs + (size_t)c.set * a.max_segs * 4;
    const int ns = a.nsegs[c.set];
    const bool rf32 = self_slot >= 0 && is_mesh(a, c.env, self_slot);
    bool hit = false;
    for (int i = c.lane; i < ns; i += 64) {
        const double sax = segs[i * 4 + 0], saz = segs[i * 4 + 1], sbx = segs[i * 4 + 2], sbz = segs[i * 4 + 3];
        const double abx = sbx - sax, abz = sbz - saz;
        const double apx = x - sax, apz = z - saz;
        const double dap = apx * abx + apz * abz;
        const double dab = abx * abx + abz * abz;
        double t = dap / dab;
        t = t < 0.0 ? 0.0 : (t > 1.0 ? 1.0 : t);
        const double cx = sax + t * abx, cz = saz + t * abz;
        const double dx = cx - x, dz = cz - z;
        hit |= sqrt(dx * dx + dz * dz) < radius;
    }
    if (ballot(hit)) return -1;
    for (int base = 0; base < a.E; base += 64) {
        const int slot = base + c.lane;
        bool h = false;
        const int kind = slot < a.E && slot != self_slot ? a.ekind[(size_t)slot * a.N + c.env] : MW_ENT_NONE;
        if (kind != MW_ENT_NONE) {
            const double dx = ent_pos(c, slot, 0) - x, dz = ent_pos(c, slot, 2) - z;
// ... 120 lines not shown
        c.cpos[0] = cp[0]; c.cpos[1] = cp[1]; c.cpos[2] = cp[2];
        c.cdir = c.dir;
    }
}

struct SubStep {
    double rew;
    int tm, tr;
    int remove_slot;
    bool ran;
    bool clean;
};

__device__ inline void trace_store(const MwArgs &a, const mw_plan_trace &t, int row, int env, double px, double py, double pz, double dir, int carry,
                                   int live, const double *cpos)
{
    const size_t r = (size_t)row * a.N + env;
    if (t.agent_pos) { t.agent_pos[r * 3 + 0] = px; t.agent_pos[r * 3 + 1] = py; t.agent_pos[r * 3 + 2] = pz; }
    if (t.agent_dir) t.agent_dir[r] = dir;
    if (t.carrying) t.carrying[r] = carry;
    if (t.ent_pos) {
        const int s = t.ent_slot;
        const bool held = live == s;
        t.ent_pos[r * 3 + 0] = held ? cpos[0] : a.epos[((size_t)0 * a.E + s) * a.N + env];
        t.ent_pos[r * 3 + 1] = held ? cpos[1] : a.epos[((size_t)1 * a.E + s) * a.N + env];
        t.ent_pos[r * 3 + 2] = held ? cpos[2] : a.epos[((size_t)2 * a.E + s) * a.N + env];
    }
}
__device__ inline void trace_fill(const MwArgs &a, const mw_plan_trace &t, int src, int k0, int k1, int env)
{
    if (k0 >= k1) return;
    const size_t N = (size_t)a.N, s = (size_t)src * N + env;
    if (t.agent_pos) {
        const double x = t.agent_pos[s * 3 + 0], y = t.agent_pos[s * 3 + 1], z = t.agent_pos[s * 3 + 2];
        for (int k = k0; k < k1; ++k) { double *d = t.agent_pos + ((size_t)k * N + env) * 3; d[0] = x; d[1] = y; d[2] = z; }
    }
    if (t.agent_dir) {
        const double v = t.agent_dir[s];
        for (int k = k0; k < k1; ++k) t.agent_dir[(size_t)k * N + env] = v;
    }
    if (t.carrying) {
        const int32_t v = t.carrying[s];
        for (int k = k0; k < k1; ++k) t.carrying[(size_t)k * N + env] = v;
    }
    if (t.ent_pos) {
        const double x = t.ent_pos[s * 3 + 0], y = t.ent_pos[s * 3 + 1], z = t.ent_pos[s * 3 + 2];
        for (int k = k0; k < k1; ++k) { double *d = t.ent_pos + ((size_t)k * N + env) * 3; d[0] = x; d[1] = y; d[2] = z; }
    }
}

template <bool PER_LANE, bool REPEAT = false, bool TRACE = false>
__device__ inline SubStep step_env(const MwArgs &a, int env, int lane, bool writer, const int32_t *__restrict__ actions,
                                float *__restrict__ reward, uint8_t *__restrict__ term, uint8_t *__restrict__ trunc,
                                unsigned char *gen_ws, int *s_claim, const mw_plan_trace *trace = nullptr, int trace_row = 0)
{
    StepCtx c{a, env, lane, a.shared_geom ? 0 : env, 0, 0, 0, 0, 0, -1, -1, {0, 0, 0}, 0};
    c.px = a.ax[env]; c.py = a.ay[env]; c.pz = a.az[env]; c.dir = a.adir[env];
    c.cam_height = a.cam[env];
    c.carry = a.carry[env];
    if (c.carry >= 0) {
        const int k = c.carry;
        c.cpos[0] = ent_pos(c, k, 0); c.cpos[1] = ent_pos(c, k, 1); c.cpos[2] = ent_pos(c, k, 2);
        c.cdir = a.edir[(size_t)k * a.N + env];
        c.live = k;
    }
    const double o_px = c.px, o_py = c.py, o_pz = c.pz, o_dir = c.dir, o_cpos[3] = {c.cpos[0], c.cpos[1], c.cpos[2]}, o_cdir = c.cdir;
    const int o_carry = c.carry;
    const int o_pending = a.pending_remove[env];
    const uint32_t o_epoch = a.fc_epoch[env];
    bool same = false;
    int remove_slot = -1;
    int tm = 0, tr = 0;
    double rew_out = 0.0;
    bool clean_out = false;
    const bool pend = a.autoreset == MW_AUTORESET_NEXT_STEP && a.reset_pending[env] != 0;

    if (!pend) {
        const int step_count = a.step[env] + 1;
        int picked = a.picked[env];
        double fwd_step = a.fwd.def, fwd_drift = a.drift.def, turn_step = a.turn.def;
        mw::Rng rng{};
        bool drew = false;
        if (a.step_override) {
            fwd_step = a.step_override[(size_t)env * 3 + 0];
            fwd_drift = a.step_override[(size_t)env * 3 + 1];
            turn_step = a.step_override[(size_t)env * 3 + 2];
        } else if (a.domain_rand) {
            rng = mw::rng_load(a.rng, a.N, env);
            fwd_step = mw::rng_uniform(rng, a.fwd.lo, a.fwd.hi);
            fwd_drift = mw::rng_uniform(rng, a.drift.lo, a.drift.hi);
            turn_step = mw::rng_uniform(rng, a.turn.lo, a.turn.hi);
            drew = true;
        }
        const int action = actions[env];
        switch (action) {
        case 2: move_agent<PER_LANE>(c, fwd_step, fwd_drift); break;
        case 3: move_agent<PER_LANE>(c, -fwd_step, fwd_drift); break;
        case 0: turn_agent<PER_LANE>(c, turn_step); break;
        case 1: turn_agent<PER_LANE>(c, -turn_step); break;
        case 4: {
            const mw::SinCos sc = mw::sincos_det(c.dir);
            const double tx = c.px + sc.c * 1.5 * a.agent_radius;
            const double tz = c.pz + (-sc.s) * 1.5 * a.agent_radius;
            const int hit = intersect<PER_LANE>(c, -1, tx, tz, 1.2 * a.agent_radius);
            if (c.carry < 0 && hit > 0 && hit <= a.E && !a.estatic[(size_t)(hit - 1) * a.N + env]) {
                const int k = hit - 1;
                c.cpos[0] = ent_pos(c, k, 0); c.cpos[1] = ent_pos(c, k, 1); c.cpos[2] = ent_pos(c, k, 2);
                c.cdir = a.edir[(size_t)k * a.N + env];
                c.carry = k;
// ... 53 lines not shown
            if (health > 0) rew = 2.0; else { rew = -100.0; tm = 1; }
        }
        if (REPEAT) rew_out = rew;
        same = same_bits(c.px, o_px) && same_bits(c.py, o_py) && same_bits(c.pz, o_pz) && same_bits(c.dir, o_dir) && c.carry == o_carry &&
               (c.live < 0 || (same_bits(c.cpos[0], o_cpos[0]) && same_bits(c.cpos[1], o_cpos[1]) && same_bits(c.cpos[2], o_cpos[2]) && same_bits(c.cdir, o_cdir)));
        if (PER_LANE) __builtin_amdgcn_wave_barrier();
        if (writer) {
            if (drew) mw::rng_store(a.rng, a.N, env, rng);
            if (!REPEAT) {
                reward[env] = (float)rew;
                term[env] = (uint8_t)tm;
                trunc[env] = (uint8_t)tr;
            }
            a.step[env] = step_count;
            a.picked[env] = picked;
            if (!PER_LANE && a.task == MW_TASK_COLLECT) a.health[env] = health;
            a.ax[env] = c.px; a.ay[env] = c.py; a.az[env] = c.pz; a.adir[env] = c.dir;
            if (c.live >= 0) {
                a.epos[((size_t)0 * a.E + c.live) * a.N + env] = c.cpos[0];
                a.epos[((size_t)1 * a.E + c.live) * a.N + env] = c.cpos[1];
                a.epos[((size_t)2 * a.E + c.live) * a.N + env] = c.cpos[2];
                a.edir[(size_t)c.live * a.N + env] = c.cdir;
            }
            a.carry[env] = remove_slot >= 0 ? -1 : c.carry;
            if (TRACE) trace_store(a, *trace, trace_row, env, c.px, c.py, c.pz, c.dir, remove_slot >= 0 ? -1 : c.carry, c.live, c.cpos);
            if ((tm | tr) && a.autoreset != MW_AUTORESET_OFF && a.generator != MW_GEN_NONE) {
                mw::keep_final_info(a, env);
                if (a.autoreset == MW_AUTORESET_NEXT_STEP) a.reset_pending[env] = 1;
            }
        }
    } else if (writer && !REPEAT) {
        reward[env] = 0.0f;
        term[env] = 0;
        trunc[env] = 0;
    } else if (TRACE && writer) {
        trace_store(a, *trace, trace_row, env, c.px, c.py, c.pz, c.dir, c.carry, c.live, c.cpos);
    }
    bool installed = false;
    if (a.generator != MW_GEN_NONE && (pend || (a.autoreset == MW_AUTORESET_SAME_STEP && (tm | tr)))) {
        installed = true;
        if (PER_LANE) {
            if (writer) mw::install_next_world<true>(a, env, 0, gen_ws, nullptr);
            __threadfence();
            __builtin_amdgcn_wave_barrier();
        } else {
            mw::install_next_world<false>(a, env, lane, gen_ws, s_claim);
        }
        c.px = a.ax[env]; c.py = a.ay[env]; c.pz = a.az[env]; c.dir = a.adir[env];
        c.carry = -1; c.live = -1;
        remove_slot = -1;
        if (pend && writer) a.reset_pending[env] = 0;
    }

    if (writer) {
        const bool clean = same && !pend && !installed && remove_slot < 0 && o_pending == -1 && a.task != MW_TASK_COLLECT;
        if (REPEAT) clean_out = clean; else { a.frame_clean[env] = clean ? 1 : 0; a.fc_source[env] = 0; }
        const bool parted = pend || installed || o_pending != -1 || c.carry != o_carry;
        if (parted) a.fc_epoch[env] = o_epoch + 1u;
        if (!REPEAT) store_frame_key(a, env, c.px, c.py, c.pz, c.dir, c.carry, o_epoch + (parted ? 1u : 0u), c.cpos[0], c.cpos[1], c.cpos[2], c.cdir);
        a.pending_remove[env] = remove_slot;
    }
    return SubStep{rew_out, tm, tr, remove_slot, !pend, clean_out};
}

template <bool PER_LANE, bool PLAN = false, bool TRACE = false>
__device__ inline void step_env_repeat(const MwArgs &a, int env, int lane, bool writer, const int32_t *__restrict__ actions, int repeat,
                                       float *__restrict__ reward, uint8_t *__restrict__ term, uint8_t *__restrict__ trunc,
                                       int32_t *__restrict__ nsteps, float *__restrict__ step_reward, bool frameless, unsigned char *gen_ws,
                                       int *s_claim, const mw_plan_trace *trace = nullptr)
{
    double sum = 0.0;
    int n = 0, tm = 0, tr = 0;
    bool clean = true, active = true;
    int rows = 0;
    for (int k = 0; k < repeat; ++k) {
        if (!ballot(active)) break;
        float rew_k = 0.0f;
        if (active) {
            const SubStep s = step_env<PER_LANE, true, TRACE>(a, env, lane, writer, PLAN ? actions + (size_t)k * a.N : actions, reward, term, trunc, gen_ws, s_claim,
                                                              trace, k);
            if (s.ran) {
                sum += s.rew;
                ++n;
                tm = s.tm; tr = s.tr;
                clean = clean && s.clean;
                if (PLAN) rew_k = (float)s.rew;
            }
            active = s.ran && !(tm | tr) && k + 1 < repeat;
            if ((active || (PLAN && frameless)) && writer && s.remove_slot >= 0) {
                if (a.task == MW_TASK_COLLECT) {
                    mw::collect_respawn(a, env, a.shared_geom ? 0 : env, s.remove_slot, a.ax[env], a.az[env]);
                    a.pending_remove[env] = -1;
                } else {
                    a.ekind[(size_t)s.remove_slot * a.N + env] = MW_ENT_NONE;
                    a.pending_remove[env] = MW_REMOVE_APPLIED;
                }
            }
        } else if (TRACE && writer) {
            trace_fill(a, *trace, k - 1, k, k + 1, env);
        }
        if (PLAN) {
            if (writer && step_reward) step_reward[(size_t)k * a.N + env] = rew_k;
            rows = k + 1;
        }
        __threadfence_block();
        __builtin_amdgcn_wave_barrier();
    }
    if (writer) {
        if (PLAN && step_reward)
            for (int k = rows; k < repeat; ++k) step_reward[(size_t)k * a.N + env] = 0.0f;
        if (TRACE) trace_fill(a, *trace, rows - 1, rows, repeat, env);
        reward[env] = (float)sum;
        term[env] = (uint8_t)tm;
        trunc[env] = (uint8_t)tr;
        if (nsteps) nsteps[env] = n;
        a.frame_clean[env] = !(PLAN && frameless) && n > 0 && clean ? 1 : 0;
        a.fc_source[env] = 0;
        const int pr = a.pending_remove[env], k = pr >= 0 ? pr : a.carry[env], ks = k >= 0 ? k : 0;
        store_frame_key(a, env, a.ax[env], a.ay[env], a.az[env], a.adir[env], k, a.fc_epoch[env], a.epos[((size_t)0 * a.E + ks) * a.N + env],
                        a.epos[((size_t)1 * a.E + ks) * a.N + env], a.epos[((size_t)2 * a.E + ks) * a.N + env], a.edir[(size_t)ks * a.N + env]);
    }
}

}

#ifndef MW_K1_MODE
#define MW_K1_MODE 0
#endif
#define MW_K1_ROW MW_CAT(MW_K1_ROW_, MW_K1_MODE)
#define MW_K1_PARAMS MW_K1_ROW(MW_K1_PARAMS_OF)
#define MW_K1_NAME(form) MW_KERNEL_NAME(MW_CAT(MW_K1_ROW(MW_K1_STEM), form))
#if MW_K1_MODE == 0
#define MW_K1_STEP(PER_LANE, env, lane, writer, ws, claim) step_env<PER_LANE>(a, env, lane, writer, actions, reward, term, trunc, ws, claim)
#elif MW_K1_MODE == 1
#define MW_K1_STEP(PER_LANE, env, lane, writer, ws, claim) \
    step_env_repeat<PER_LANE>(a, env, lane, writer, actions, repeat, reward, term, trunc, nsteps, nullptr, false, ws, claim)
#elif MW_K1_MODE == 2
#define MW_K1_STEP(PER_LANE, env, lane, writer, ws, claim) \
    step_env_repeat<PER_LANE, true>(a, env, lane, writer, actions, horizon, reward, term, trunc, nsteps, step_reward, frameless != 0, ws, claim)
#elif MW_K1_MODE == 3
#define MW_K1_STEP(PER_LANE, env, lane, writer, ws, claim) \
    step_env_repeat<PER_LANE, true, true>(a, env, lane, writer, actions, horizon, reward, term, trunc, nsteps, step_reward, frameless != 0, ws, claim, &trace)
#else
#error "MW_K1_MODE is not a mode of mw_kernels.h's K1 table"
#endif
```

miniworld_amd/csrc/mw_setup_dense.hip:

```cpp
#include "mw_setup_common.h"
#include "mw_kernels.h"


extern "C" __global__ __launch_bounds__(64) __attribute__((amdgpu_waves_per_eu(1, 2))) void MW_K1_NAME(_dense)(
    MW_K1_PARAMS)
{
    __shared__ unsigned char gen_ws[MW_GEN_WS_BYTES];
    const int lane = threadIdx.x;
    const int L = lanes_per_env;
    const int epw = 64 / L;
    const int el = (int)(((uint32_t)lane * ((65536u + (uint32_t)L - 1u) / (uint32_t)L)) >> 16);
    const int slot = lane - el * L;
    const int env_blocks = (a.N + epw - 1) / epw;
    if ((int)blockIdx.x >= env_blocks) {
        mw::refill_spares(a, (int)blockIdx.x - env_blocks, lane, gen_ws);
        return;
    }
    const int env = (int)blockIdx.x * epw + el;
    if (el >= epw || env >= a.N) return;
    MW_K1_STEP(true, env, lane, slot == 0, gen_ws, nullptr);
}
```

miniworld_amd/engine.py:

```python
from __future__ import annotations

import ctypes as C
import os
import subprocess
import sys

import numpy as np

_CSRC = os.path.join(os.path.dirname(os.path.abspath(__file__)), "csrc")
PRODUCT_PATH = os.path.join(_CSRC, "libmwengine.so")
LIB_PATH = os.environ.get("MW_ENGINE_LIB") or PRODUCT_PATH

ABI_VERSION = 4
MAX_REPEAT = 256
MAX_PLAN = MAX_REPEAT
MAX_STACK = 16
STACK_PAD_RESET, STACK_PAD_ZERO = 0, 1
SNAPF_DEPTH, SNAPF_STACK = 1, 2
ENT_NONE, ENT_BOX, ENT_MESH, ENT_FRAME = 0, 1, 2, 3
POLY_ENTITY = 0x100
POLY_XF = 0x200
POLY_QUAD = 0x400
TASK_NONE, TASK_GOTO, TASK_PICKUP, TASK_PUTNEXT, TASK_SIDEWALK, TASK_SIGN, TASK_COLLECT = 0, 1, 2, 3, 4, 5, 6
GEN_NONE, GEN_HALLWAY, GEN_ONEROOM, GEN_PICKUP, GEN_MAZE, GEN_PROGRAM = 0, 1, 2, 3, 4, 5
# ... 156 lines not shown
    "mw_set_step_params": _sig(vp, vp),
    "mw_set_gen_program": _sig(vp, P(MwGenProgram), vp, vp, vp, vp, i32, vp, i32),
    "mw_reset": _sig(vp, vp, vp, vp),
    "mw_reset_where": _sig(vp, vp, vp, vp),
    "mw_set_reset_seeds": _sig(vp, vp),
    "mw_step": _sig(vp, vp, vp, vp, vp, vp, vp, vp),
    "mw_step_repeat": _sig(vp, vp, i32, vp, vp, vp, vp, vp, vp, vp),
    "mw_step_plan": _sig(vp, vp, i32, vp, vp, vp, vp, vp, vp, vp, vp),
    "mw_step_plan_trace": _sig(vp, vp, i32, vp, vp, vp, vp, vp, vp, vp, P(MwPlanTrace), vp),
    "mw_render": _sig(vp, vp, vp, vp),
    "mw_render_top": _sig(vp, vp, vp, i32, vp),
    "mw_render_view": _sig(vp, i32, i32, i32, i32, i32, vp, vp, vp),
    "mw_visible_ents": _sig(vp, i32, i32, vp, vp),
    "mw_set_obs_layout": _sig(vp, i32),
    "mw_set_final_obs": _sig(vp, vp, vp),
    "mw_set_frame_stack": _sig(vp, i32, i32, vp, vp),
    "mw_stack_refresh": _sig(vp, vp, vp),
    "mw_stack_window": _sig(vp, P(i32), P(i64)),
    "mw_snapshot_bytes": _sig(vp, i32, ret=i64),
    "mw_snapshot_save": _sig(vp, vp, i32, vp, i32, vp),
    "mw_snapshot_load": _sig(vp, vp, vp, i32, vp, i32, i32, vp),
    "mw_snapshot_frames_bytes": _sig(vp, i32, i32, ret=i64),
    "mw_snapshot_save_frames": _sig(vp, vp, i32, vp, vp, vp, i32, i32, vp),
    "mw_snapshot_load_frames": _sig(vp, vp, vp, i32, vp, i32, i32, i32, vp, vp, vp),
    "mw_snapshot_save_at": _sig(vp, vp, vp, i32, vp, i32, vp),
    "mw_snapshot_save_frames_at": _sig(vp, vp, vp, i32, vp, vp, vp, i32, i32, vp),
    "mw_snapshot_load_where": _sig(vp, vp, vp, vp, i32, i32, vp),
    "mw_snapshot_load_frames_where": _sig(vp, vp, vp, vp, i32, i32, i32, vp, vp, vp),
    "mw_nav_build": _sig(vp, P(MwNavParams), vp, vp, vp, vp),
    "mw_nav_query": _sig(vp, P(MwNavParams), vp, vp, vp, vp, vp, vp, vp),
    "mw_debug_set_nav_passes": _sig(vp, vp),
    "mw_ray_cast": _sig(vp, P(MwRayParams), vp, vp, vp, vp, vp, vp, vp, vp),
    "mw_debug_set_ray_form": _sig(vp, C.c_int),
    "mw_seen_update": _sig(vp, P(MwNavParams), P(C.c_double), i32, vp, vp, vp, vp, vp, vp),
    "mw_debug_set_launch_shape": _sig(vp, C.c_int, C.c_int, C.c_int, C.c_int),
    "mw_pcg64_draws": _sig(C.c_uint64, i32, vp, vp),
    "mw_selftest_rcp": _sig(vp, vp, vp),
    "mw_selftest_div": _sig(vp, vp),
    "mw_selftest_sort": _sig(vp, vp, i32, vp),
    "mw_selftest_q": _sig(vp, vp),
    "mw_selftest_sincosf": _sig(vp, C.c_uint64, vp),
    "mw_check": _sig(vp, vp),
    "mw_kernel_time_ms": _sig(vp, i32, P(C.c_double), P(C.c_double), P(i64)),
    "mw_raster_path": _sig(vp),
    "mw_get_info": _sig(vp, vp, vp, i32, vp),
    "mw_get_final_info": _sig(vp, vp, vp, vp),
    "mw_get_reset_pending": _sig(vp, vp, vp),
    "mw_set_frame_reuse": _sig(vp, i32),
    "mw_get_frame_clean": _sig(vp, vp, vp),
    "mw_set_frame_cache": _sig(vp, i32),
    "mw_get_frame_source": _sig(vp, vp, vp),
    "mw_get_frame_plan": _sig(vp, vp, i64, vp, vp),
    "mw_get_geom_built": _sig(vp, vp, vp),
    "mw_get_list_lengths": _sig(vp, i32, i32, vp, vp),
    "mw_debug_set_mesh_frame_seq": _sig(vp, C.c_uint32),
    "mw_debug_get_slow_heads": _sig(vp, vp, vp),
}
EXPORTS = list(SIGNATURES)

_said = set()


def build_library(force: bool = False) -> str:
    if LIB_PATH != PRODUCT_PATH:
        if LIB_PATH not in _said:
            _said.add(LIB_PATH)
            print(f"miniworld_amd: MW_ENGINE_LIB is set: loading {LIB_PATH} as it is, not building {PRODUCT_PATH}", file=sys.stderr)
        return LIB_PATH
    srcs = [os.path.join(_CSRC, f) for f in os.listdir(_CSRC) if f.endswith((".hip", ".h"))]
    srcs.append(os.path.join(_CSRC, "..", "..", "include", "mwengine.h"))
    stale = (not os.path.exists(LIB_PATH)) or any(os.path.getmtime(s) > os.path.getmtime(LIB_PATH) for s in srcs)
    if force or stale:
        r = subprocess.run([os.path.join(_CSRC, "build.sh")], capture_output=True, text=True)
        if r.returncode != 0:
            raise EngineError("building libmwengine.so failed:\n" + r.stdout + r.stderr)
    return LIB_PATH


_lib = None


def load_library():
    global _lib
    if _lib is not None:
        return _lib
    import torch
    if not os.path.exists(LIB_PATH):
        raise EngineError(
            f"{LIB_PATH} not found: the HIP engine is not built (run `python -c 'import __graft_entry__ as g; "
            "g.build()'` or miniworld_amd/csrc/build.sh).  There is no CPU fallback.")
    L = C.CDLL(LIB_PATH)
    for name, (argtypes, restype) in SIGNATURES.items():
        fn = getattr(L, name)
        fn.argtypes, fn.restype = argtypes, restype
    _lib = L
    return L


def frame_reuse_allowed() -> bool:
    return os.environ.get("MW_FRAME_REUSE", "1").strip() != "0"


MAX_FRAME_CACHE = 8


def frame_cache_allowed() -> bool:
# ... 506 lines not shown
        self._dev_tensor(health, "health", torch.int32, self.N)
        self._dev_tensor(pos, "position", torch.float64, self.N * 3)

    def get_info(self, health=None, ent_pos=None, ent_slot=0):
        self._info_tensors(health, ent_pos)
        self._check(self.lib.mw_get_info(self.h, _ptr(health), _ptr(ent_pos), int(ent_slot), _stream_ptr(self.device)), "mw_get_info")

    def get_final_info(self, health=None, goal_pos=None):
        self._info_tensors(health, goal_pos)
        self._check(self.lib.mw_get_final_info(self.h, _ptr(health), _ptr(goal_pos), _stream_ptr(self.device)), "mw_get_final_info")

    def _get_bytes(self, fn, out):
        import torch
        if out is None:
            out = torch.zeros(self.N, dtype=torch.uint8, device=self.device)
        self._dev_tensor(out, fn, torch.uint8, self.N)
        self._check(getattr(self.lib, fn)(self.h, _ptr(out), _stream_ptr(self.device)), fn)
        return out

    def get_reset_pending(self, out=None):
        return self._get_bytes("mw_get_reset_pending", out)

    def set_frame_reuse(self, on: bool):
        on = bool(on) and frame_reuse_allowed()
        self._check(self.lib.mw_set_frame_reuse(self.h, int(on)), "mw_set_frame_reuse")
        self.frame_reuse = on
        return on

    def set_frame_cache(self, slots: int):
        slots = int(slots) if frame_cache_allowed() else 0
        self._check(self.lib.mw_set_frame_cache(self.h, slots), "mw_set_frame_cache")
        self.frame_cache = slots
        return slots

    def get_frame_source(self, out=None):
        return self._get_bytes("mw_get_frame_source", out)

    def get_frame_plan(self):
        N = self.N
        ordered = N <= 0xFFFF
        block = np.zeros(96 + N * (9 if ordered else 2), np.uint32)
        lengths = np.zeros(N, np.int32)
        self._check(self.lib.mw_get_frame_plan(self.h, block.ctypes.data, block.size, lengths.ctypes.data, _stream_ptr(self.device)), "mw_get_frame_plan")
        n_draw, n_copy, classes = int(block[0]), int(block[1]), int(block[2])
        packed = [int(block[32]) | int(block[33]) << 32, int(block[64]) | int(block[65]) << 32]
        counts = [(packed[c >> 2] >> (16 * (c & 3))) & 0xFFFF for c in range(8)] if classes else []
        if classes:
            draw = np.concatenate([block[96 + N * (1 + c):96 + N * (1 + c) + min(counts[c], N)] for c in reversed(range(8))])
        else:
            draw = block[96 + N:96 + N + min(n_draw, N)].copy()
        return {"n_draw": n_draw, "n_copy": n_copy, "classes": classes, "class_counts": counts, "draw": draw,
                "copy": block[96:96 + min(n_copy, N)].copy(), "lengths": lengths, "block": block}

    def get_geom_built(self):
        out = np.zeros(self.N, np.uint8)
        self._check(self.lib.mw_get_geom_built(self.h, out.ctypes.data, _stream_ptr(self.device)), "mw_get_geom_built")
        return out

    def get_frame_clean(self, out=None):
        return self._get_bytes("mw_get_frame_clean", out)

    def list_lengths(self):
        out = np.zeros(self.N, np.int32)
        self._check(self.lib.mw_get_list_lengths(self.h, 0, self.N, out.ctypes.data, _stream_ptr(self.device)), "mw_get_list_lengths")
        return out

    def raster_path(self):
        return int(self.lib.mw_raster_path(self.h))

    def kernel_time_ms(self, reset=0):
        r, s, n = C.c_double(), C.c_double(), C.c_int64()
        self._check(self.lib.mw_kernel_time_ms(self.h, reset, C.byref(r), C.byref(s), C.byref(n)), "mw_kernel_time_ms")
        return r.value, s.value, n.value



def default_ranges() -> dict:
    return {
        "sky_color": ([0.25, 0.82, 1.0], [0.1, 0.1, 0.1], [1.0, 1.0, 1.0]),
        "light_pos": ([0, 2.5, 0], [-40, 2.5, -40], [40, 5, 40]),
        "light_color": ([0.7, 0.7, 0.7], [0.45, 0.45, 0.45], [0.8, 0.8, 0.8]),
        "light_ambient": ([0.45, 0.45, 0.45], [0.35, 0.35, 0.35], [0.55, 0.55, 0.55]),
        "obj_color_bias": ([0, 0, 0], [-0.2, -0.2, -0.2], [0.2, 0.2, 0.2]),
        "forward_step": (0.15, 0.12, 0.17),
        "forward_drift": (0.0, -0.05, 0.05),
        "turn_step": (15.0, 10.0, 20.0),
        "cam_pitch": (0.0, -5.0, 5.0),
        "cam_fov_y": (60.0, 55.0, 65.0),
        "cam_height": (1.5, 1.45, 1.55),
        "cam_fwd_disp": (0.0, -0.05, 0.10),
    }


def fill_ranges(cfg: MwConfig, ranges: dict | None = None):
    r = default_ranges() if ranges is None else ranges
    for name in ("forward_step", "forward_drift", "turn_step", "cam_pitch", "cam_fov_y", "cam_height", "cam_fwd_disp"):
        setattr(cfg, name, MwRange.of(*r[name]))
    for name in ("sky_color", "light_pos", "light_color", "light_ambient", "obj_color_bias"):
        d, lo, hi = r[name]
        arr = getattr(cfg, name)
        for k in range(3):
            arr[k] = MwRange.of(d[k], lo[k], hi[k])
    cfg.max_forward_step = float(r["forward_step"][2])
```

Measured before the change: 18.51 million.

## Hoist frame-cache verdict into step kernel for geometry and plan reuse

The step kernel now computes each env's frame key, matches it against the frame-cache metadata, and stores a one-byte verdict per env (source slot, victim, build flag). The geometry kernel's deal mask and the frame-plan kernel then read this verdict instead of recomputing cleanliness and cache matches from frame_clean, fc_key and meta. The aim is to remove redundant key loads and cache-matching work from two later kernels. In exchange the step kernel does extra work and needs an extra verdict buffer, and the path only applies when the step_prologue policy conditions hold.

```diff
diff --git a/include/mwengine.h b/include/mwengine.h
--- a/include/mwengine.h
+++ b/include/mwengine.h
@@ -312,6 +312,8 @@
 int mw_get_frame_plan(mw_engine *e, uint32_t *host_plan, int64_t words, int32_t *host_lengths, void *stream);
 int mw_get_geom_built(mw_engine *e, uint8_t *host_out, void *stream);
 
+int mw_get_step_prologue(mw_engine *e);
+
 int mw_get_list_lengths(mw_engine *e, int32_t first_env, int32_t count, int32_t *host_out, void *stream);
 
 int mw_debug_set_mesh_frame_seq(mw_engine *e, uint32_t seq);
diff --git a/miniworld_amd/csrc/mw_engine.h b/miniworld_amd/csrc/mw_engine.h
--- a/miniworld_amd/csrc/mw_engine.h
+++ b/miniworld_amd/csrc/mw_engine.h
@@ -122,6 +122,9 @@
     int plan_cur = 0;
     bool geom_deal = true;
     uint8_t *d_geom_built = nullptr;
+    bool step_prologue = true;
+    bool step_prologue_last = false;
+    uint8_t *d_pro_verdict = nullptr;
     bool plan_made = false;
     struct {
         int depth = 0, pad = 0, layout = 0, cur = 0;
diff --git a/miniworld_amd/csrc/mw_engine.hip b/miniworld_amd/csrc/mw_engine.hip
--- a/miniworld_amd/csrc/mw_engine.hip
+++ b/miniworld_amd/csrc/mw_engine.hip
@@ -200,6 +200,7 @@
     ALLOC(e->d_plan[0], MW_PLAN_WORDS(N, frame_plan_ordered(N))); ALLOC(e->d_plan[1], MW_PLAN_WORDS(N, frame_plan_ordered(N)));
     ALLOC(e->stack.flags, 2 * (size_t)N);
     ALLOC(e->d_geom_built, (size_t)N);
+    ALLOC(e->d_pro_verdict, (size_t)N);
     ALLOC(e->d_mask, N); ALLOC(e->d_step_override, 3 * (size_t)N);
 #ifdef MW_PERF_HOOKS
     if (getenv("MW_K1_PROF")) ALLOC(a.k1_prof, MW_K1_PROF_SLOTS * (size_t)N);
@@ -239,6 +240,7 @@
     if (const char *s = getenv("MW_K2Q")) e->use_k2q = atoi(s) != 0;
     if (const char *s = getenv("MW_GENERIC_RASTER")) e->generic_raster = atoi(s) != 0;
     if (const char *s = getenv("MW_GEOM_DEAL")) e->geom_deal = atoi(s) != 0;
+    if (const char *s = getenv("MW_STEP_PROLOGUE")) e->step_prologue = atoi(s) != 0;
     e->k2q_ok = k2q_ok(cfg->msaa, a.W, a.H, mw_rasterq_lds_bytes(cfg->msaa == 4 ? 4 : 8, a.W, a.H, a.n_tiles, 1));
     {
         e->snap_cfg = {E, cfg->max_polys, cfg->max_segs, cfg->shared_geometry ? 1 : 0, cfg->task, cfg->generator, cfg->rng_mode, e->spare_mode ? 1 : 0,
@@ -763,6 +765,12 @@
     return MW_OK;
 }
 
+int mw_get_step_prologue(mw_engine *e)
+{
+    if (!e) return fail(e, MW_E_INVALID, "mw_get_step_prologue: null argument");
+    return e->step_prologue_last ? 1 : 0;
+}
+
 int mw_get_geom_built(mw_engine *e, uint8_t *host_out, void *stream)
 {
     if (!e || !host_out) return fail(e, MW_E_INVALID, "mw_get_geom_built: null argument");
diff --git a/miniworld_amd/csrc/mw_engine_frame.hip b/miniworld_amd/csrc/mw_engine_frame.hip
--- a/miniworld_amd/csrc/mw_engine_frame.hip
+++ b/miniworld_amd/csrc/mw_engine_frame.hip
@@ -157,41 +157,51 @@
     bool plans;
     RasterPath p;
     MeshFrame mf;
+    MwStepPro pro;
 };
 
 bool side_refills(const mw_engine *e) { return e->spare_mode && e->cfg.generator == MW_GEN_MAZE; }
 
-void launch_k1(mw_engine *e, const MwArgs &ak, const Call &c, bool frameless)
+void launch_k1(mw_engine *e, const MwArgs &ak, const Call &c, bool frameless, const MwStepPro &pro)
 {
     const int N = e->cfg.num_envs;
     const int refill_blocks = (e->spare_mode && !side_refills(e)) ? (N + 63) / 64 : 0;
     const int lanes = dense_lanes_of(e);
     const dim3 grid(env_blocks(N, lanes) + refill_blocks);
     if (c.horizon > 0 && c.trace)
-        hipLaunchKernelGGL(MW_K1(e, lanes, mw_step_trace), grid, dim3(64), 0, c.st, ak, lanes, c.actions, c.reward, c.term, c.trunc, c.horizon, c.nsteps, c.step_reward,
+        hipLaunchKernelGGL(MW_K1(e, lanes, mw_step_trace), grid, dim3(64), 0, c.st, ak, lanes, c.actions, c.reward, c.term, c.trunc, pro, c.horizon, c.nsteps, c.step_reward,
                            frameless ? 1 : 0, *c.trace);
     else if (c.horizon > 0)
-        hipLaunchKernelGGL(MW_K1(e, lanes, mw_step_plan), grid, dim3(64), 0, c.st, ak, lanes, c.actions, c.reward, c.term, c.trunc, c.horizon, c.nsteps, c.step_reward,
+        hipLaunchKernelGGL(MW_K1(e, lanes, mw_step_plan), grid, dim3(64), 0, c.st, ak, lanes, c.actions, c.reward, c.term, c.trunc, pro, c.horizon, c.nsteps, c.step_reward,
                            frameless ? 1 : 0);
-    else if (c.repeat > 0) hipLaunchKernelGGL(MW_K1(e, lanes, mw_step_repeat), grid, dim3(64), 0, c.st, ak, lanes, c.actions, c.reward, c.term, c.trunc, c.repeat, c.nsteps);
-    else hipLaunchKernelGGL(MW_K1(e, lanes, mw_step_setup), grid, dim3(64), 0, c.st, ak, lanes, c.actions, c.reward, c.term, c.trunc);
+    else if (c.repeat > 0) hipLaunchKernelGGL(MW_K1(e, lanes, mw_step_repeat), grid, dim3(64), 0, c.st, ak, lanes, c.actions, c.reward, c.term, c.trunc, pro, c.repeat, c.nsteps);
+    else hipLaunchKernelGGL(MW_K1(e, lanes, mw_step_setup), grid, dim3(64), 0, c.st, ak, lanes, c.actions, c.reward, c.term, c.trunc, pro);
+}
+
+bool frame_deals(const mw_engine *e, const Frame &f) { return geom_deals(f.plans, e->geom_deal, geom_lanes_of(e)); }
+MwStepPro step_pro_of(const mw_engine *e, const Frame &f, CallKind kind)
+{
+    const int slots = f.pol.cache ? e->fc.slots : 0;
+    if (!step_prologue(kind, dense_lanes_of(e), frame_deals(e, f), e->step_prologue, slots)) return MwStepPro{nullptr, nullptr, 0, 0};
+    return MwStepPro{e->d_pro_verdict, slots ? (const uint64_t *)e->fc.meta.get() : nullptr, slots, f.pol.reuse ? 1 : 0};
 }
 
 void launch_step_and_geometry(mw_engine *e, const Frame &f, const Call &c, CallKind kind)
 {
     const MwArgs &a = f.a; const int N = e->cfg.num_envs;
+    const MwStepPro &pro = f.pro;
     if (call_steps(kind)) {
         MwArgs ak = a;
         if (kind == CALL_TERMINAL_STEP) ak.autoreset = MW_AUTORESET_NEXT_STEP;
-        launch_k1(e, ak, c, false);
+        launch_k1(e, ak, c, false, pro);
     }
     if (kind == CALL_TERMINAL_STEP)
         hipLaunchKernelGGL(mw_final_list_kernel, dim3(1), dim3(1024), 0, f.st, N, (const uint8_t *)a.reset_pending, a.pending_remove, e->d_final_list);
     const int L = geom_lanes_of(e);
-    const bool deals = geom_deals(f.plans, e->geom_deal, L);
+    const bool deals = frame_deals(e, f);
     const int flags = f.view_flags | (deals ? MW_GEOM_DEAL | (f.pol.reuse ? MW_GEOM_REUSE : 0) : 0);
     launch(geom_kernel_of(L, e->cfg.msaa), f.list, dim3(env_blocks(N, L)), dim3(64), 0, f.st, a, flags, e->cfg.msaa, L, N,
-           deals && f.pol.cache ? (const uint64_t *)e->fc.meta.get() : nullptr, deals && f.pol.cache ? e->fc.slots : 0, e->d_geom_built);
+           deals && f.pol.cache ? (const uint64_t *)e->fc.meta.get() : nullptr, deals && f.pol.cache ? e->fc.slots : 0, e->d_geom_built, pro);
     if (call_steps(kind) && e->cfg.task == MW_TASK_COLLECT)
         hipLaunchKernelGGL(MW_BY_STREAM(e, mw_collect_respawn), dim3((N + 63) / 64), dim3(64), 0, f.st, a);
 }
@@ -243,7 +253,8 @@
     e->plan_made = true;
     hipLaunchKernelGGL(mw_frame_plan_kernel, dim3((N + MW_PLAN_ENVS - 1) / MW_PLAN_ENVS), dim3(64), 0, st, N, f.pol.reuse ? 1 : 0, (const uint8_t *)a.frame_clean,
                        (const uint64_t *)a.fc_key, f.pol.cache ? (const uint64_t *)e->fc.meta.get() : nullptr, f.pol.cache ? e->fc.slots : 0,
-                       frame_plan_ordered(N) ? (const int32_t *)a.nvis : nullptr, a.fc_source, plan, next);
+                       frame_plan_ordered(N) ? (const int32_t *)a.nvis : nullptr, a.fc_source, plan, next,
+                       (const uint8_t *)f.pro.verdict);
     return plan;
 }
 
@@ -307,8 +318,10 @@
                                           e->fc.slots > 0 && e->fc.frames, path.path, e->reset_seeds != nullptr});
     frames_stale(e);
     const int N = e->cfg.num_envs;
-    Frame f{e->args, view_flags, kind == CALL_LIST_PASS ? e->d_final_list : nullptr, d_obs, d_depth, st, pol, false, path, {}};
+    Frame f{e->args, view_flags, kind == CALL_LIST_PASS ? e->d_final_list : nullptr, d_obs, d_depth, st, pol, false, path, {}, {}};
     f.plans = frame_plans(pol, path.path, f.list != nullptr, N);
+    f.pro = step_pro_of(e, f, kind);
+    e->step_prologue_last = f.pro.verdict != nullptr;
     if (pol.cache) {
         if (d_depth && !e->fc.depth) {
             if (const int rc = dev_alloc(e, e->fc.depth, (size_t)N * e->fc.slots * f.a.W * f.a.H, false)) return rc;
@@ -383,7 +396,7 @@
     const int N = e->cfg.num_envs;
     MwArgs a = e->args;
     a.step_override = e->use_step_override ? e->d_step_override : nullptr;
-    launch_k1(e, a, c, true);
+    launch_k1(e, a, c, true, MwStepPro{nullptr, nullptr, 0, 0});
     if (side_refills(e))
         if (const int rc = launch_side_refill(e, c.st)) return rc;
     if (e->stack.depth) {
@@ -550,7 +563,7 @@
     b.W = width; b.H = height;
     b.tiles_x = tiles_across(width); b.tiles_y = tiles_down(height); b.n_tiles = b.tiles_x * b.tiles_y;
     b.env_base = env;
-    hipLaunchKernelGGL(geom_kernel_of(64, msaa).plain, dim3(1), dim3(64), 0, st, b, view_flags, msaa, 64, 1, (const uint64_t *)nullptr, 0, (uint8_t *)nullptr);
+    hipLaunchKernelGGL(geom_kernel_of(64, msaa).plain, dim3(1), dim3(64), 0, st, b, view_flags, msaa, 64, 1, (const uint64_t *)nullptr, 0, (uint8_t *)nullptr, MwStepPro{nullptr, nullptr, 0, 0});
     if (const int rc = e->have_meshes ? grow(e, e->mp.view_keys, e->mp.view_keys_bytes, (size_t)width * height * msaa * 4, 1) : MW_OK) return rc;
     if (const int rc = launch_generic(e, b, env, 1, msaa, dim3(128), d_out, d_depth, MW_OBS_HWC_U8, nullptr, st)) return rc;
     HIP_TRY(e, hipGetLastError());
@@ -579,7 +592,7 @@
     b.env_base = first_env;
     {
         const int L = geom_lanes_of(e);
-        hipLaunchKernelGGL(geom_kernel_of(L, e->cfg.msaa).plain, dim3(env_blocks(count, L)), dim3(64), 0, st, b, 4, e->cfg.msaa, L, count, (const uint64_t *)nullptr, 0, (uint8_t *)nullptr);
+        hipLaunchKernelGGL(geom_kernel_of(L, e->cfg.msaa).plain, dim3(env_blocks(count, L)), dim3(64), 0, st, b, 4, e->cfg.msaa, L, count, (const uint64_t *)nullptr, 0, (uint8_t *)nullptr, MwStepPro{nullptr, nullptr, 0, 0});
     }
     if (!e->visible_attr_set) {
         HIP_TRY(e, hipFuncSetAttribute((const void *)mw_visible_kernel, hipFuncAttributeMaxDynamicSharedMemorySize, (int)lds));
diff --git a/miniworld_amd/csrc/mw_engine_kernels.hip b/miniworld_amd/csrc/mw_engine_kernels.hip
--- a/miniworld_amd/csrc/mw_engine_kernels.hip
+++ b/miniworld_amd/csrc/mw_engine_kernels.hip
@@ -57,7 +57,8 @@
 
 extern "C" __global__ __launch_bounds__(64) void mw_frame_plan_kernel(int N, int reuse, const uint8_t *__restrict__ frame_clean, const uint64_t *__restrict__ key,
                                                                      const uint64_t *__restrict__ meta, int slots, const int32_t *__restrict__ nvis,
-                                                                     uint8_t *__restrict__ frame_source, uint32_t *__restrict__ plan, uint32_t *__restrict__ next)
+                                                                     uint8_t *__restrict__ frame_source, uint32_t *__restrict__ plan, uint32_t *__restrict__ next,
+                                                                     const uint8_t *__restrict__ verdict)
 {
     const int lane = (int)threadIdx.x, env = (int)blockIdx.x * MW_PLAN_ENVS + lane;
     const bool ordered = nvis != nullptr;
@@ -70,7 +71,13 @@
     const bool on = env < N;
     uint32_t v = MW_SRC_CLEAN;
     uint32_t cls = 0u;
-    if (on) {
+    if (on && verdict) {
+        const uint8_t kv = verdict[env];
+        const int32_t len = ordered ? nvis[env] : 0;
+        v = mw_verdict_frame(kv);
+        frame_source[env] = (uint8_t)v;
+        cls = mw_plan_cost_class(len);
+    } else if (on) {
         const bool clean = frame_clean[env] != 0;
         const int32_t len = ordered ? nvis[env] : 0;
         uint32_t match = 0u, header = 0u;
diff --git a/miniworld_amd/csrc/mw_geom.hip b/miniworld_amd/csrc/mw_geom.hip
--- a/miniworld_amd/csrc/mw_geom.hip
+++ b/miniworld_amd/csrc/mw_geom.hip
@@ -198,7 +198,8 @@
 }
 
 template <bool BIG, int SFIX, bool SUB = false>
-__device__ inline void geom_body(const MwArgs &a, int view_flags, int S_, int L, int n_env, const uint64_t *fc_meta, int fc_slots, uint8_t *built, const int32_t *__restrict__ list = nullptr)
+__device__ inline void geom_body(const MwArgs &a, int view_flags, int S_, int L, int n_env, const uint64_t *fc_meta, int fc_slots, uint8_t *built, const uint8_t *verdict,
+                                 const int32_t *__restrict__ list = nullptr)
 {
     const int S = SFIX ? SFIX : S_;
     struct ClipSlot { mwgl::ClipVert l[2][MWGL_MAX_CLIP_VERTS]; float pad[4]; };
@@ -221,11 +222,12 @@
     const unsigned long long tstart = KGP_ON ? __builtin_readcyclecounter() : 0ull;
     const unsigned long long rt_start = KGP_ON ? __builtin_amdgcn_s_memrealtime() : 0ull;
     [[maybe_unused]] unsigned long long ts[4] = {0, 0, 0, 0};
-    [[maybe_unused]] int kp_nocc = 0, kp_nkept = 0, kp_nclip = 0;
+    [[maybe_unused]] int kp_nocc = 0, kp_nkept = 0, kp_nclip = 0, kp_envclip = 0;
     [[maybe_unused]] unsigned long long kp_clip = 0, kp_emit = 0, kp_e_shfl = 0, kp_e_setup = 0, kp_e_write = 0;
     const int lane = threadIdx.x;
     const int epw = 64 / L, sub = lane & (L - 1), grp = lane / L;
     const bool deal = !BIG && !SUB && (view_flags & MW_GEOM_DEAL) != 0;
+    const bool hoisted = deal && verdict != nullptr;
     int rel, env;
     bool live;
     constexpr bool kPoseAhead = !BIG && !SUB;
@@ -254,7 +256,8 @@
             for (int i = 0; i < 4; ++i) ahead[13 + i] = a.cam[(size_t)i * a.N + ge];
         }
         uint64_t mask;
-        if (deal) mask = deal_mask(a.frame_clean, a.pending_remove, a.fc_key, fc_meta, fc_slots, (view_flags & MW_GEOM_REUSE) != 0, a.env_base + 64 * g, n_env - 64 * g, lane, reinterpret_cast<uint4 *>(&s_clip[0]));
+        if (hoisted) mask = __ballot(mine < n_env && mw_verdict_build(verdict[a.env_base + min(mine, n_env - 1)]));
+        else if (deal) mask = deal_mask(a.frame_clean, a.pending_remove, a.fc_key, fc_meta, fc_slots, (view_flags & MW_GEOM_REUSE) != 0, a.env_base + 64 * g, n_env - 64 * g, lane, reinterpret_cast<uint4 *>(&s_clip[0]));
         else mask = __ballot(mine < n_env);
         const bool want = ((mask >> lane) & 1ull) != 0ull;
         if (deal && i == 0 && mine < n_env && !want) built[a.env_base + mine] = 0;
@@ -943,6 +946,7 @@
         const uint64_t cmask = __ballot(clipped);
         const uint64_t below = (1ull << lane) - 1ull;
         const int n_clip = (int)__popcll((unsigned long long)cmask);
+        if (KGP_ON) kp_envclip += (int)__popcll((unsigned long long)((cmask >> (grp * L)) & (L == 64 ? ~0ull : (1ull << L) - 1ull)));
         const bool keep_lists = n_clip <= kClipSlots;
         const uint32_t cm_union = va.clipmask | vb.clipmask | vc.clipmask;
         const bool par = !__any(clipped && __popc(cm_union) == 6);
@@ -1146,6 +1150,7 @@
         pp[10] = (unsigned long long)np; pp[11] = (unsigned long long)npd; pp[12] = (unsigned long long)count; pp[13] = (unsigned long long)n_rounds;
         pp[14] = (unsigned long long)kp_nocc; pp[15] = (unsigned long long)kp_nkept;
         pp[16] = ts[0] - tp[0]; pp[17] = ts[1] - ts[0]; pp[18] = ts[2] - ts[1]; pp[19] = ts[3] - ts[2];
+        pp[31] = (unsigned long long)kp_envclip;
     }
     if (ent_pre && my_mesh_j >= 0 && live) {
         const int nb = total_boxes < 64 ? total_boxes : 64;
@@ -1206,8 +1211,8 @@
 #define MW_GEOM_OCC
 #endif
 #define MW_GEOM_PAIR(stem, bounds, ...)                                                                                        \
-    extern "C" __global__ bounds void stem##_kernel(MW_GEOM_ARGS) { geom_body<__VA_ARGS__, false>(a, view_flags, S, L, n_env, fc_meta, fc_slots, built); } \
-    extern "C" __global__ bounds void stem##_sub_kernel(MW_GEOM_ARGS, const int32_t *list) { geom_body<__VA_ARGS__, true>(a, view_flags, S, L, n_env, fc_meta, fc_slots, built, list); }
+    extern "C" __global__ bounds void stem##_kernel(MW_GEOM_ARGS) { geom_body<__VA_ARGS__, false>(a, view_flags, S, L, n_env, fc_meta, fc_slots, built, pro.verdict); } \
+    extern "C" __global__ bounds void stem##_sub_kernel(MW_GEOM_ARGS, const int32_t *list) { geom_body<__VA_ARGS__, true>(a, view_flags, S, L, n_env, fc_meta, fc_slots, built, pro.verdict, list); }
 MW_GEOM_PAIR(mw_geom, __launch_bounds__(64) MW_GEOM_OCC, false, 8)
 MW_GEOM_PAIR(mw_geom_big, __launch_bounds__(64) MW_GEOM_OCC, true, 8)
 MW_GEOM_PAIR(mw_geom_any, __launch_bounds__(64), false, 0)
diff --git a/miniworld_amd/csrc/mw_kernels.h b/miniworld_amd/csrc/mw_kernels.h
--- a/miniworld_amd/csrc/mw_kernels.h
+++ b/miniworld_amd/csrc/mw_kernels.h
@@ -1,6 +1,7 @@
 #pragma once
 #include "mw_device.h"
 #include "mw_frame_plan.h"
+#include "mw_step_prologue.h"
 #include "mw_snapshot.h"
 #include "mw_snapframes.h"
 #include "mw_state_view.h"
@@ -25,7 +26,7 @@
 #define MW_K1_STEM(stem, ...) stem
 #define MW_K1_PARAMS_OF(stem, ...) __VA_ARGS__
 #define MW_K1_ARGS MwArgs a, int lanes_per_env, const int32_t *__restrict__ actions, float *__restrict__ reward, \
-                   uint8_t *__restrict__ term, uint8_t *__restrict__ trunc
+                   uint8_t *__restrict__ term, uint8_t *__restrict__ trunc, MwStepPro pro
 #define MW_K1_ROW_0(X) X(mw_step_setup, MW_K1_ARGS)
 MW_K1_ROW_0(MW_K1_DECLARE);
 #define MW_K1_REPEAT_ARGS MW_K1_ARGS, int repeat, int32_t *__restrict__ nsteps
@@ -48,7 +49,7 @@
 
 #define MW_GEOM_DEAL 8
 #define MW_GEOM_REUSE 16
-#define MW_GEOM_ARGS MwArgs a, int view_flags, int S, int L, int n_env, const uint64_t *fc_meta, int fc_slots, uint8_t *built
+#define MW_GEOM_ARGS MwArgs a, int view_flags, int S, int L, int n_env, const uint64_t *fc_meta, int fc_slots, uint8_t *built, MwStepPro pro
 MW_KERNEL_PAIR(mw_geom, MW_GEOM_ARGS);
 MW_KERNEL_PAIR(mw_geom_big, MW_GEOM_ARGS);
 MW_KERNEL_PAIR(mw_geom_any, MW_GEOM_ARGS);
@@ -149,7 +150,8 @@
 #define MW_PLAN_ENVS 64
 extern "C" __global__ void mw_frame_plan_kernel(int N, int reuse, const uint8_t *__restrict__ frame_clean, const uint64_t *__restrict__ key,
                                                 const uint64_t *__restrict__ meta, int slots, const int32_t *__restrict__ nvis,
-                                                uint8_t *__restrict__ frame_source, uint32_t *__restrict__ plan, uint32_t *__restrict__ next);
+                                                uint8_t *__restrict__ frame_source, uint32_t *__restrict__ plan, uint32_t *__restrict__ next,
+                                                const uint8_t *__restrict__ verdict);
 
 #define MW_SV_THREADS 256
 #define MW_SV_ENVS (MW_SV_THREADS / 64)
diff --git a/miniworld_amd/csrc/mw_policy.h b/miniworld_amd/csrc/mw_policy.h
--- a/miniworld_amd/csrc/mw_policy.h
+++ b/miniworld_amd/csrc/mw_policy.h
@@ -145,6 +145,10 @@
 {
     return plans && enabled && lanes < 64;
 }
+inline bool step_prologue(CallKind kind, int dense_lanes, bool deals, bool enabled, int slots)
+{
+    return kind == CALL_STEP && dense_lanes > 0 && deals && enabled && slots <= dense_lanes;
+}
 inline bool frame_plan_ordered(int N)
 {
     return N <= 0xFFFF;
diff --git a/miniworld_amd/csrc/mw_setup.hip b/miniworld_amd/csrc/mw_setup.hip
--- a/miniworld_amd/csrc/mw_setup.hip
+++ b/miniworld_amd/csrc/mw_setup.hip
@@ -15,5 +15,5 @@
         return;
     }
     const int lane = threadIdx.x & 63;
-    MW_K1_STEP(false, a.env_base + (int)blockIdx.x, lane, lane == 0, gen_ws, &s_claim);
+    MW_K1_STEP(false, a.env_base + (int)blockIdx.x, lane, lane, lane == 0, gen_ws, &s_claim);
 }
diff --git a/miniworld_amd/csrc/mw_setup_common.h b/miniworld_amd/csrc/mw_setup_common.h
--- a/miniworld_amd/csrc/mw_setup_common.h
+++ b/miniworld_amd/csrc/mw_setup_common.h
@@ -3,6 +3,7 @@
 #include "mw_math.h"
 #include "mw_rng.h"
 #include "mw_gen.h"
+#include "mw_step_prologue.h"
 
 namespace {
 
@@ -22,17 +23,56 @@
 
 __device__ inline bool same_bits(double x, double y) { return __double_as_longlong(x) == __double_as_longlong(y); }
 
+__device__ inline void frame_key_words(double px, double py, double pz, double dir, int carry, uint32_t epoch, double cx, double cy, double cz, double cdir,
+                                       uint64_t (&k)[MW_FC_KEY_WORDS])
+{
+    auto bits = [](double v) { return (uint64_t)__double_as_longlong(v); };
+    const bool c = carry >= 0;
+    k[0] = bits(px); k[1] = bits(py); k[2] = bits(pz); k[3] = bits(dir);
+    k[4] = (uint64_t)(uint32_t)carry | ((uint64_t)epoch << 32);
+    k[5] = c ? bits(cx) : 0ull; k[6] = c ? bits(cy) : 0ull; k[7] = c ? bits(cz) : 0ull; k[8] = c ? bits(cdir) : 0ull;
+    k[9] = 1ull;
+}
 __device__ inline void store_frame_key(const MwArgs &a, int env, double px, double py, double pz, double dir, int carry, uint32_t epoch,
                                        double cx, double cy, double cz, double cdir)
 {
+    uint64_t w[MW_FC_KEY_WORDS];
+    frame_key_words(px, py, pz, dir, carry, epoch, cx, cy, cz, cdir, w);
     ulonglong2 *k = reinterpret_cast<ulonglong2 *>(a.fc_key + (size_t)env * MW_FC_KEY_WORDS);
-    auto bits = [](double v) { return (unsigned long long)__double_as_longlong(v); };
-    const bool c = carry >= 0;
-    k[0] = make_ulonglong2(bits(px), bits(py));
-    k[1] = make_ulonglong2(bits(pz), bits(dir));
-    k[2] = make_ulonglong2((unsigned long long)(uint32_t)carry | ((unsigned long long)epoch << 32), c ? bits(cx) : 0ull);
-    k[3] = make_ulonglong2(c ? bits(cy) : 0ull, c ? bits(cz) : 0ull);
-    k[4] = make_ulonglong2(c ? bits(cdir) : 0ull, 1ull);
+#pragma unroll
+    for (int i = 0; i < MW_FC_KEY_WORDS / 2; ++i) k[i] = make_ulonglong2(w[2 * i], w[2 * i + 1]);
+}
+
+
+struct ProAhead { ulonglong2 k[MW_FC_KEY_WORDS / 2]; uint32_t header; };
+__device__ inline void pro_request(const MwStepPro &pro, int env, int sub, ProAhead &p)
+{
+#pragma unroll
+    for (int i = 0; i < MW_FC_KEY_WORDS / 2; ++i) p.k[i] = make_ulonglong2(0ull, 0ull);
+    p.header = 0u;
+    if (pro.meta && pro.slots > 0) {
+        const uint64_t *row = static_cast<const uint64_t *>(__builtin_assume_aligned(pro.meta + (size_t)env * MW_FC_META_WORDS(pro.slots), 16));
+        const ulonglong2 *q = reinterpret_cast<const ulonglong2 *>(row + 2 + MW_FC_KEY_WORDS * (sub < pro.slots ? sub : pro.slots - 1));
+        p.header = (uint32_t)row[0];
+#pragma unroll
+        for (int i = 0; i < MW_FC_KEY_WORDS / 2; ++i) p.k[i] = q[i];
+    }
+}
+
+__device__ inline uint32_t pro_match(const MwStepPro &pro, const ProAhead &p, const uint64_t (&key)[MW_FC_KEY_WORDS], int lane, int sub)
+{
+    uint64_t slot_key[MW_FC_KEY_WORDS];
+#pragma unroll
+    for (int i = 0; i < MW_FC_KEY_WORDS / 2; ++i) { slot_key[2 * i] = p.k[i].x; slot_key[2 * i + 1] = p.k[i].y; }
+    const bool eq = pro.meta != nullptr && sub < pro.slots && mw_fc_key_equal(slot_key, key);
+    const uint64_t m = ballot(eq);
+    return (uint32_t)(m >> (lane - sub)) & ((1u << pro.slots) - 1u);
+}
+
+__device__ inline void pro_store(const MwStepPro &pro, int env, bool clean, int pending, uint32_t match, uint32_t header)
+{
+    const uint32_t v = mw_frame_verdict(clean, pro.reuse != 0, match, header, pro.meta ? pro.slots : 0);
+    pro.verdict[env] = mw_verdict_of(v, pending);
 }
 
 
@@ -259,9 +299,13 @@
 template <bool PER_LANE, bool REPEAT = false, bool TRACE = false>
 __device__ inline SubStep step_env(const MwArgs &a, int env, int lane, bool writer, const int32_t *__restrict__ actions,
                                 float *__restrict__ reward, uint8_t *__restrict__ term, uint8_t *__restrict__ trunc,
-                                unsigned char *gen_ws, int *s_claim, const mw_plan_trace *trace = nullptr, int trace_row = 0)
+                                unsigned char *gen_ws, int *s_claim, const MwStepPro &pro, int sub, const mw_plan_trace *trace = nullptr, int trace_row = 0)
 {
     StepCtx c{a, env, lane, a.shared_geom ? 0 : env, 0, 0, 0, 0, 0, -1, -1, {0, 0, 0}, 0};
+    [[maybe_unused]] ProAhead pro_row;
+    if constexpr (PER_LANE && !REPEAT) {
+        if (pro.verdict) pro_request(pro, env, sub, pro_row);
+    }
     c.px = a.ax[env]; c.py = a.ay[env]; c.pz = a.az[env]; c.dir = a.adir[env];
     c.cam_height = a.cam[env];
     c.carry = a.carry[env];
@@ -421,13 +465,23 @@
         if (pend && writer) a.reset_pending[env] = 0;
     }
 
+    const bool clean = same && !pend && !installed && remove_slot < 0 && o_pending == -1 && a.task != MW_TASK_COLLECT;
+    const bool parted = pend || installed || o_pending != -1 || c.carry != o_carry;
     if (writer) {
-        const bool clean = same && !pend && !installed && remove_slot < 0 && o_pending == -1 && a.task != MW_TASK_COLLECT;
         if (REPEAT) clean_out = clean; else { a.frame_clean[env] = clean ? 1 : 0; a.fc_source[env] = 0; }
-        const bool parted = pend || installed || o_pending != -1 || c.carry != o_carry;
         if (parted) a.fc_epoch[env] = o_epoch + 1u;
         if (!REPEAT) store_frame_key(a, env, c.px, c.py, c.pz, c.dir, c.carry, o_epoch + (parted ? 1u : 0u), c.cpos[0], c.cpos[1], c.cpos[2], c.cdir);
         a.pending_remove[env] = remove_slot;
+    }
+    if constexpr (PER_LANE && !REPEAT) {
+        if (pro.verdict) {
+            uint64_t key[MW_FC_KEY_WORDS];
+            frame_key_words(c.px, c.py, c.pz, c.dir, c.carry, o_epoch + (parted ? 1u : 0u), c.cpos[0], c.cpos[1], c.cpos[2], c.cdir, key);
+            const uint32_t match = pro_match(pro, pro_row, key, lane, sub);
+            if (writer) {
+                pro_store(pro, env, clean, remove_slot, match, pro_row.header);
+            }
+        }
     }
     return SubStep{rew_out, tm, tr, remove_slot, !pend, clean_out};
 }
@@ -436,8 +490,12 @@
 __device__ inline void step_env_repeat(const MwArgs &a, int env, int lane, bool writer, const int32_t *__restrict__ actions, int repeat,
                                        float *__restrict__ reward, uint8_t *__restrict__ term, uint8_t *__restrict__ trunc,
                                        int32_t *__restrict__ nsteps, float *__restrict__ step_reward, bool frameless, unsigned char *gen_ws,
-                                       int *s_claim, const mw_plan_trace *trace = nullptr)
-{
+                                       int *s_claim, const MwStepPro &pro, int sub, const mw_plan_trace *trace = nullptr)
+{
+    [[maybe_unused]] ProAhead pro_row;
+    if constexpr (PER_LANE) {
+        if (pro.verdict) pro_request(pro, env, sub, pro_row);
+    }
     double sum = 0.0;
     int n = 0, tm = 0, tr = 0;
     bool clean = true, active = true;
@@ -447,7 +505,7 @@
         float rew_k = 0.0f;
         if (active) {
             const SubStep s = step_env<PER_LANE, true, TRACE>(a, env, lane, writer, PLAN ? actions + (size_t)k * a.N : actions, reward, term, trunc, gen_ws, s_claim,
-                                                              trace, k);
+                                                              pro, sub, trace, k);
             if (s.ran) {
                 sum += s.rew;
                 ++n;
@@ -489,6 +547,17 @@
         store_frame_key(a, env, a.ax[env], a.ay[env], a.az[env], a.adir[env], k, a.fc_epoch[env], a.epos[((size_t)0 * a.E + ks) * a.N + env],
                         a.epos[((size_t)1 * a.E + ks) * a.N + env], a.epos[((size_t)2 * a.E + ks) * a.N + env], a.edir[(size_t)ks * a.N + env]);
     }
+    if constexpr (PER_LANE) {
+        if (pro.verdict) {
+            const int pr = a.pending_remove[env], k = pr >= 0 ? pr : a.carry[env], ks = k >= 0 ? k : 0;
+            const double pose[4] = {a.ax[env], a.ay[env], a.az[env], a.adir[env]};
+            uint64_t key[MW_FC_KEY_WORDS];
+            frame_key_words(pose[0], pose[1], pose[2], pose[3], k, a.fc_epoch[env], a.epos[((size_t)0 * a.E + ks) * a.N + env],
+                            a.epos[((size_t)1 * a.E + ks) * a.N + env], a.epos[((size_t)2 * a.E + ks) * a.N + env], a.edir[(size_t)ks * a.N + env], key);
+            const uint32_t match = pro_match(pro, pro_row, key, lane, sub);
+            if (writer) pro_store(pro, env, !(PLAN && frameless) && n > 0 && clean, pr, match, pro_row.header);
+        }
+    }
 }
 
 }
@@ -500,16 +569,16 @@
 #define MW_K1_PARAMS MW_K1_ROW(MW_K1_PARAMS_OF)
 #define MW_K1_NAME(form) MW_KERNEL_NAME(MW_CAT(MW_K1_ROW(MW_K1_STEM), form))
 #if MW_K1_MODE == 0
-#define MW_K1_STEP(PER_LANE, env, lane, writer, ws, claim) step_env<PER_LANE>(a, env, lane, writer, actions, reward, term, trunc, ws, claim)
+#define MW_K1_STEP(PER_LANE, env, lane, sub, writer, ws, claim) step_env<PER_LANE>(a, env, lane, writer, actions, reward, term, trunc, ws, claim, pro, sub)
 #elif MW_K1_MODE == 1
-#define MW_K1_STEP(PER_LANE, env, lane, writer, ws, claim) \
-    step_env_repeat<PER_LANE>(a, env, lane, writer, actions, repeat, reward, term, trunc, nsteps, nullptr, false, ws, claim)
+#define MW_K1_STEP(PER_LANE, env, lane, sub, writer, ws, claim) \
+    step_env_repeat<PER_LANE>(a, env, lane, writer, actions, repeat, reward, term, trunc, nsteps, nullptr, false, ws, claim, pro, sub)
 #elif MW_K1_MODE == 2
-#define MW_K1_STEP(PER_LANE, env, lane, writer, ws, claim) \
-    step_env_repeat<PER_LANE, true>(a, env, lane, writer, actions, horizon, reward, term, trunc, nsteps, step_reward, frameless != 0, ws, claim)
+#define MW_K1_STEP(PER_LANE, env, lane, sub, writer, ws, claim) \
+    step_env_repeat<PER_LANE, true>(a, env, lane, writer, actions, horizon, reward, term, trunc, nsteps, step_reward, frameless != 0, ws, claim, pro, sub)
 #elif MW_K1_MODE == 3
-#define MW_K1_STEP(PER_LANE, env, lane, writer, ws, claim) \
-    step_env_repeat<PER_LANE, true, true>(a, env, lane, writer, actions, horizon, reward, term, trunc, nsteps, step_reward, frameless != 0, ws, claim, &trace)
+#define MW_K1_STEP(PER_LANE, env, lane, sub, writer, ws, claim) \
+    step_env_repeat<PER_LANE, true, true>(a, env, lane, writer, actions, horizon, reward, term, trunc, nsteps, step_reward, frameless != 0, ws, claim, pro, sub, &trace)
 #else
 #error "MW_K1_MODE is not a mode of mw_kernels.h's K1 table"
 #endif
diff --git a/miniworld_amd/csrc/mw_setup_dense.hip b/miniworld_amd/csrc/mw_setup_dense.hip
--- a/miniworld_amd/csrc/mw_setup_dense.hip
+++ b/miniworld_amd/csrc/mw_setup_dense.hip
@@ -18,5 +18,5 @@
     }
     const int env = (int)blockIdx.x * epw + el;
     if (el >= epw || env >= a.N) return;
-    MW_K1_STEP(true, env, lane, slot == 0, gen_ws, nullptr);
+    MW_K1_STEP(true, env, lane, slot, slot == 0, gen_ws, nullptr);
 }
diff --git a/miniworld_amd/csrc/mw_step_prologue.h b/miniworld_amd/csrc/mw_step_prologue.h
--- /dev/null
+++ b/miniworld_amd/csrc/mw_step_prologue.h
@@ -0,0 +1,31 @@
+#pragma once
+#include <stdint.h>
+
+#include "mw_hd.h"
+#include "mw_frame_plan.h"
+
+#define MW_VERDICT_BUILD 0x80u
+MW_HD uint8_t mw_verdict_encode(uint32_t source, uint32_t victim, bool build)
+{
+    return (uint8_t)((source & 0xFu) | (victim & 0x7u) << 4 | (build ? MW_VERDICT_BUILD : 0u));
+}
+MW_HD uint32_t mw_verdict_source(uint8_t v) { return v & 0xFu; }
+MW_HD uint32_t mw_verdict_victim(uint8_t v) { return (v >> 4) & 0x7u; }
+MW_HD bool mw_verdict_build(uint8_t v) { return (v & MW_VERDICT_BUILD) != 0u; }
+MW_HD uint8_t mw_verdict_of(uint32_t frame_verdict, int pending_remove)
+{
+    const uint32_t src = frame_verdict & 0xFFu;
+    const bool drawn = src == (uint32_t)MW_SRC_DRAWN;
+    return mw_verdict_encode(src, drawn ? frame_verdict >> 8 : 0u, drawn || pending_remove >= 0);
+}
+MW_HD uint32_t mw_verdict_frame(uint8_t v)
+{
+    const uint32_t src = mw_verdict_source(v);
+    return src | (src >= (uint32_t)MW_SRC_SLOT(0) ? src - (uint32_t)MW_SRC_SLOT(0) : mw_verdict_victim(v)) << 8;
+}
+
+struct MwStepPro {
+    uint8_t *verdict;
+    const uint64_t *meta;
+    int32_t slots, reuse;
+};
diff --git a/miniworld_amd/engine.py b/miniworld_amd/engine.py
--- a/miniworld_amd/engine.py
+++ b/miniworld_amd/engine.py
@@ -232,6 +232,7 @@
     "mw_get_frame_source": _sig(vp, vp, vp),
     "mw_get_frame_plan": _sig(vp, vp, i64, vp, vp),
     "mw_get_geom_built": _sig(vp, vp, vp),
+    "mw_get_step_prologue": _sig(vp),
     "mw_get_list_lengths": _sig(vp, i32, i32, vp, vp),
     "mw_debug_set_mesh_frame_seq": _sig(vp, C.c_uint32),
     "mw_debug_get_slow_heads": _sig(vp, vp, vp),
@@ -844,6 +845,12 @@
         return {"n_draw": n_draw, "n_copy": n_copy, "classes": classes, "class_counts": counts, "draw": draw,
                 "copy": block[96:96 + min(n_copy, N)].copy(), "lengths": lengths, "block": block}
 
+    def step_prologue_ran(self) -> bool:
+        r = self.lib.mw_get_step_prologue(self.h)
+        if r < 0:
+            self._check(r, "mw_get_step_prologue")
+        return r == 1
+
     def get_geom_built(self):
         out = np.zeros(self.N, np.uint8)
         self._check(self.lib.mw_get_geom_built(self.h, out.ctypes.data, _stream_ptr(self.device)), "mw_get_geom_built")
```

Result: faster. 18.71 million (median of 6 runs) (+1.1%).
